# pyani-plus/pyani-plus

Hardware: AMD Instinct MI355X
Metric: pairwise genome comparisons/sec (N x N ANI matrix) (higher is better)
Workload: dtype u64

## Files before the change

include/pyani_hip.h:

```cpp
#ifndef PYANI_HIP_H
#define PYANI_HIP_H

#include <stddef.h>
#include <stdint.h>

#ifdef __cplusplus
extern "C" {
#endif

#define PA_ABI_VERSION 5

#define PA_API __attribute__((visibility("default")))

typedef enum pa_status {
  PA_OK = 0,
  PA_E_INVALID = -1,
  PA_E_HIP = -2,
  PA_E_NOMEM = -3,
  PA_E_CAPACITY = -4,
  PA_E_NODEVICE = -5,
  PA_E_IO = -6
} pa_status;

typedef struct pa_ctx pa_ctx;

#define PA_ALIGN_BASES 64u
#define PA_MAX_K 64u

PA_API int pa_abi_version(void);
PA_API const char *pa_last_error(void);
PA_API int pa_device_count(void);
PA_API int pa_ctx_create(int device, pa_ctx **out);
PA_API void pa_ctx_destroy(pa_ctx *ctx);
PA_API int pa_ctx_set_stream(pa_ctx *ctx, void *hip_stream);
PA_API int pa_ctx_own_stream(pa_ctx *ctx);
PA_API int pa_ctx_sync(pa_ctx *ctx);
PA_API int pa_ctx_device_info(pa_ctx *ctx, char *name256, int *compute_units, uint64_t *global_mem);

PA_API int pa_dev_alloc(pa_ctx *ctx, uint64_t bytes, void **d_out);
PA_API int pa_dev_free(pa_ctx *ctx, void *d_ptr);
PA_API int pa_memcpy_h2d(pa_ctx *ctx, void *d_dst, const void *h_src, uint64_t bytes);
PA_API int pa_memcpy_d2h(pa_ctx *ctx, void *h_dst, const void *d_src, uint64_t bytes);
PA_API int pa_memset_d(pa_ctx *ctx, void *d_dst, int value, uint64_t bytes);

PA_API uint64_t pa_pack_bound(uint64_t n_text_bytes);
PA_API int pa_pack_fasta(const uint8_t *h_text, uint64_t n_text, uint32_t *h_packed, uint32_t *h_mask,
                  uint64_t cap_bases, uint64_t *n_bases, uint64_t *n_residues, uint64_t *n_records,
                  uint64_t *n_invalid);
PA_API int pa_pack_seq(const uint8_t *h_seq, uint64_t n_seq, uint32_t *h_packed, uint32_t *h_mask,
                uint64_t cap_bases, uint64_t *n_bases, uint64_t *n_invalid);

PA_API int pa_gunzip(const uint8_t *h_gz, uint64_t n_gz, uint8_t *h_out, uint64_t cap, uint64_t *n_out, int decoder);

typedef struct pa_fasta_batch pa_fasta_batch;
PA_API int pa_fasta_batch_load(const char *const *paths, uint32_t n, int threads, pa_fasta_batch **out);
PA_API int pa_fasta_batch_info(const pa_fasta_batch *batch, uint32_t i, char md5hex33[33], uint64_t *n_residues,
                        uint64_t *n_records, uint64_t *n_invalid, uint64_t *n_bases, uint64_t *n_text,
                        const char **description, const char **message, int *was_gzip);
PA_API int pa_fasta_batch_records(const pa_fasta_batch *batch, uint32_t i, const uint64_t **rec_start,
                           const uint64_t **rec_len, uint64_t *n_records);
PA_API uint64_t pa_fasta_batch_arena_bases(const pa_fasta_batch *batch);
PA_API int pa_fasta_batch_copy_arena(const pa_fasta_batch *batch, uint32_t *h_packed, uint32_t *h_mask,
                              uint64_t *h_genome_start);
PA_API void pa_fasta_batch_free(pa_fasta_batch *batch);

PA_API uint64_t pa_max_hash(uint64_t scaled);

PA_API int pa_arena_dirty(pa_ctx *ctx, const uint32_t *d_mask, uint64_t arena_bases, uint64_t *d_dirty);

PA_API int pa_sketch(pa_ctx *ctx, const uint32_t *d_packed, const uint32_t *d_mask, const uint64_t *d_dirty,
              uint64_t arena_bases, const uint64_t *h_genome_start, uint32_t n_genomes, uint32_t k, uint64_t max_hash,
              uint64_t *d_hashes, uint64_t cap_hashes, uint64_t *d_off, uint64_t *h_total);

PA_API int64_t pa_mask_runs(const uint32_t *h_mask, uint64_t arena_bases, uint64_t *h_run_start, uint64_t *h_run_len,
                            uint64_t cap);
PA_API int pa_mask_from_runs(pa_ctx *ctx, const uint64_t *h_run_start, const uint64_t *h_run_len, uint32_t n_runs,
                             uint32_t *d_mask, uint64_t arena_bases);
PA_API int pa_sketch_streamed(pa_ctx *ctx, const uint32_t *h_packed, const uint64_t *h_run_start,
                              const uint64_t *h_run_len, uint32_t n_runs, uint64_t arena_bases,
                              const uint64_t *h_genome_start, uint32_t n_genomes, uint32_t k, uint64_t max_hash,
                              uint32_t *d_packed, uint32_t *d_mask, uint64_t *d_dirty, uint64_t *d_hashes,
                              uint64_t cap_hashes, uint64_t *d_off, uint64_t *h_total);

#define PA_PAIRS_AUTO 0
#define PA_PAIRS_BITROW 1
#define PA_PAIRS_MERGE 2
#define PA_PAIRS_BITROW_HASH 3
PA_API int pa_pair_counts(pa_ctx *ctx, const uint64_t *d_hashes, const uint64_t *d_off, uint32_t n,
                   uint32_t q0, uint32_t q1, uint32_t s0, uint32_t s1, uint32_t *d_counts, int algo);
PA_API int pa_pair_counts_ex(pa_ctx *ctx, const uint64_t *d_hashes, const uint64_t *d_off, const uint64_t *h_off,
                      uint32_t n, uint32_t q0, uint32_t q1, uint32_t s0, uint32_t s1, uint32_t *d_counts, int algo);
PA_API int pa_pair_dict_prepare(pa_ctx *ctx, const uint64_t *d_subject_hashes, uint64_t n_postings);

PA_API int pa_ani(pa_ctx *ctx, const uint32_t *d_counts, const uint64_t *d_off, uint32_t q0, uint32_t q1,
           uint32_t s0, uint32_t s1, uint32_t k, double *d_identity, double *d_cov_query);
PA_API int pa_ani_host(const uint32_t *h_counts, const uint64_t *h_q_sizes, const uint64_t *h_s_sizes,
                uint32_t nq, uint32_t ns, uint32_t k, double *h_identity, double *h_cov_query,
                uint8_t *h_is_null, int symmetric, uint32_t n_threads);

PA_API int pa_sketch_bottom(pa_ctx *ctx, const uint32_t *d_packed, const uint32_t *d_mask, const uint64_t *d_dirty, uint64_t arena_bases,
                     const uint64_t *h_genome_start, uint32_t n_genomes, uint32_t k, uint32_t m, uint64_t *d_hashes,
                     uint64_t cap_hashes, uint64_t *d_off, uint64_t *h_total);
PA_API int pa_pair_mash(pa_ctx *ctx, const uint64_t *d_hashes, const uint64_t *d_off, uint32_t n, uint32_t q0, uint32_t q1,
                 uint32_t s0, uint32_t s1, uint32_t m, uint32_t *d_common, uint32_t *d_denom);
PA_API int pa_ani_mash(pa_ctx *ctx, const uint32_t *d_common, const uint32_t *d_denom, uint64_t n_pairs, uint32_t k,
                double *d_ani);

PA_API int pa_fragani(pa_ctx *ctx, const uint32_t *d_packed, const uint32_t *d_mask, uint64_t arena_bases,
               const uint64_t *h_contig_start, const uint32_t *h_contig_len, const uint32_t *h_contig_genome,
               uint32_t n_contigs, uint32_t n_genomes, uint32_t k, uint32_t frag_len, uint32_t ref0, uint32_t ref1,
               uint32_t *h_total_frags, uint32_t *h_matched, double *h_ident_sum);
#define PA_FRAGANI_REUSE_INDEX 1u
#define PA_FRAGANI_COLUMNS_ONLY 2u
PA_API int pa_fragani_ex(pa_ctx *ctx, const uint32_t *d_packed, const uint32_t *d_mask, uint64_t arena_bases,
                  const uint64_t *h_contig_start, const uint32_t *h_contig_len, const uint32_t *h_contig_genome,
                  uint32_t n_contigs, uint32_t n_genomes, uint32_t k, uint32_t frag_len, uint32_t qry0, uint32_t qry1,
                  uint32_t ref0, uint32_t ref1, uint32_t flags, uint32_t *h_total_frags, uint32_t *h_matched,
                  double *h_ident_sum);
PA_API int pa_fragani_workspace(pa_ctx *ctx, uint64_t *held_bytes, uint64_t *peak_bytes, uint64_t *cap_bytes);
PA_API int pa_fragani_set_workspace_cap(pa_ctx *ctx, uint64_t cap_bytes);
PA_API int64_t pa_text_ambiguous(const uint8_t *h_text, uint64_t n_text, int fasta, uint64_t *h_pos, uint8_t *h_byte,
                                 uint64_t cap);
PA_API int64_t pa_fasta_batch_ambiguous(const pa_fasta_batch *batch, uint64_t *h_pos, uint8_t *h_byte, uint64_t cap);
PA_API int pa_fragani_set_ambiguous(pa_ctx *ctx, const uint32_t *d_packed, const uint64_t *h_pos, const uint8_t *h_byte,
                                    uint64_t n);
PA_API int pa_fragani_sketch(pa_ctx *ctx, const uint32_t *d_packed, const uint32_t *d_mask, uint64_t arena_bases,
                      const uint64_t *h_contig_start, const uint32_t *h_contig_len, const uint32_t *h_contig_genome,
                      uint32_t n_contigs, uint32_t n_genomes, uint32_t k, uint32_t window, uint32_t *h_hash,
                      uint32_t *h_wpos, uint32_t *h_contig, uint64_t cap, uint64_t *n_out);
PA_API int pa_fragani_window(uint32_t k, uint32_t frag_len);
PA_API int pa_fragani_tables(uint32_t k, uint32_t s_max, uint32_t *h_min_hits, uint32_t *h_min_shared);
PA_API double pa_fragani_identity(uint32_t shared, uint32_t s, uint32_t k);
PA_API int64_t pa_fasta_records(const uint8_t *h_text, uint64_t n_text, uint64_t *h_rec_start, uint64_t *h_rec_len,
                         uint64_t cap);

PA_API int pa_write_sigs(uint32_t n_files, const char *const *paths, const char *const *heads, const char *const *mids,
                         const char *const *tails, uint32_t ksize, const uint64_t *h_mins, const uint64_t *h_off,
                         uint32_t n_threads);

#define PA_SIG_UNHANDLED 1
typedef struct pa_sig_batch pa_sig_batch;
PA_API int pa_read_sigs(const char *const *paths, uint32_t n, uint32_t ksize, uint64_t max_hash, uint32_t n_threads,
                        pa_sig_batch **out);
PA_API int pa_sig_batch_info(const pa_sig_batch *batch, uint32_t i, uint64_t *n_mins, const char **message);
PA_API int pa_sig_batch_copy(const pa_sig_batch *batch, uint64_t *h_mins, uint64_t *h_off);
PA_API void pa_sig_batch_free(pa_sig_batch *batch);

PA_API int pa_write_comparisons_json(const char *path, const char *prefix, const char *suffix,
                              const char *const *q_hashes, uint32_t nq, const char *const *s_hashes, uint32_t ns,
                              const double *h_identity, const double *h_cov_query, const uint8_t *h_is_null);

PA_API int pa_append_comparisons_json(const char *path, const char *suffix, int file_has_rows,
                               const char *const *q_hashes, uint32_t nq, const char *const *s_hashes, uint32_t ns,
                               const double *h_identity, const double *h_cov_query, const uint8_t *h_is_null);

PA_API int pa_append_comparisons_json_ex(const char *path, const char *suffix, int file_has_rows,
                                  const char *const *q_hashes, uint32_t nq, const char *const *s_hashes, uint32_t ns,
                                  const double *h_identity, const double *h_cov_query, const uint8_t *h_is_null,
                                  const int64_t *h_aln_length, const int64_t *h_sim_errors);

PA_API int pa_round_sig6(double *h_values, uint64_t n);

PA_API uint32_t pa_host_cpu_budget(void);

PA_API int pa_sqlite_insert_comparisons(const char *database, int64_t configuration_id, const char *uname_system,
                                        const char *uname_release, const char *uname_machine,
                                        const char *const *query_hashes, uint32_t n_queries,
                                        const char *const *subject_hashes, uint32_t n_subjects,
                                        const double *h_identity, const double *h_cov_query, const uint8_t *h_is_null,
                                        uint64_t *rows_inserted);

PA_API int pa_sqlite_insert_comparisons_ex(const char *database, int64_t configuration_id, const char *uname_system,
                                           const char *uname_release, const char *uname_machine,
                                           const char *const *query_hashes, uint32_t n_queries,
                                           const char *const *subject_hashes, uint32_t n_subjects,
                                           const double *h_identity, const double *h_cov_query, const uint8_t *h_is_null,
                                           const int64_t *h_aln_length, const int64_t *h_sim_errors,
                                           uint64_t *rows_inserted);

typedef struct pa_msa pa_msa;
PA_API int pa_msa_load(const char *path, int threads, pa_msa **out);
PA_API int pa_msa_info(const pa_msa *msa, uint32_t *n_records, uint64_t *max_len, char md5hex33[33], uint64_t *h_hist256);
PA_API int pa_msa_record(const pa_msa *msa, uint32_t i, const char **title, uint64_t *title_len, uint64_t *length);
PA_API int pa_msa_copy_rows(const pa_msa *msa, uint32_t r0, uint32_t r1, uint64_t row_stride, uint8_t *h_rows);
PA_API void pa_msa_free(pa_msa *msa);
PA_API uint64_t pa_msa_plane_words(uint32_t n_rows, uint64_t n_cols, uint32_t bits);
PA_API int pa_msa_pack(pa_ctx *ctx, const uint8_t *d_rows, uint64_t row_stride, uint32_t row0, uint32_t n_chunk_rows, uint32_t n_rows,
                       uint64_t n_cols, const uint8_t *h_code256, uint32_t bits, uint32_t *d_planes, uint32_t *d_nongap);
PA_API int pa_msa_pair_counts(pa_ctx *ctx, const uint32_t *d_planes, uint32_t n_rows, uint64_t n_cols, uint32_t bits, uint32_t q0,
                              uint32_t q1, uint32_t s0, uint32_t s1, int symmetric, uint32_t *d_match, uint32_t *d_both);
PA_API int pa_msa_metrics(const uint32_t *h_match, const uint32_t *h_both, const uint64_t *h_nq, const uint64_t *h_ns, uint64_t n_pairs,
                          double *h_identity, int64_t *h_aln_length, int64_t *h_sim_errors, double *h_cov_query,
                          double *h_cov_subject, uint32_t n_threads);
PA_API int pa_append_msa_json(const char *path, const char *suffix, int file_has_rows, const char *const *hashes, uint32_t n_hashes,
                              const uint32_t *q_idx, const uint32_t *s_idx, uint64_t n_rows, const double *identity,
                              const int64_t *aln_length, const int64_t *sim_errors, const double *cov_query, const double *cov_subject);

#define PA_AGG_MIN 0
#define PA_AGG_MAX 1
#define PA_AGG_MEAN 2
typedef struct pa_cliques pa_cliques;
PA_API int pa_classify_edges(pa_ctx *ctx, const double *d_score, const double *d_cov, uint32_t n, int agg_score, int agg_cov,
                             double cov_min, uint64_t cap_edges, uint32_t *d_i, uint32_t *d_j, double *d_edge_score,
                             double *d_edge_cov, uint64_t *n_edges);
PA_API int pa_classify_edges_host(const double *h_score, const double *h_cov, uint32_t n, int agg_score, int agg_cov, double cov_min,
                                  uint64_t cap_edges, uint32_t *h_i, uint32_t *h_j, double *h_edge_score, double *h_edge_cov,
                                  uint64_t *n_edges);
PA_API int pa_classify_tani_host(const double *h_hadamard, uint64_t n_cells, double *h_score);
PA_API int pa_classify_cliques(uint32_t n, uint64_t n_edges, const uint32_t *h_i, const uint32_t *h_j, const double *h_edge_score,
                               const double *h_edge_cov, pa_cliques **out);
PA_API int pa_cliques_info(const pa_cliques *cl, uint64_t *n_rows, uint64_t *n_members);
PA_API int pa_cliques_copy(const pa_cliques *cl, uint32_t *n_nodes, double *max_cov, double *min_score, double *max_score,
                           uint8_t *present, uint64_t *member_off, uint32_t *members);
PA_API void pa_cliques_free(pa_cliques *cl);

#define PA_PROF_KMER_HASH 0
#define PA_PROF_SKETCH_SORT 1
#define PA_PROF_PAIR_DICT 2
#define PA_PROF_PAIR_COUNT 3
#define PA_PROF_ANI 4
#define PA_PROF_FRAG_INDEX 5
#define PA_PROF_FRAG_SEED 6
#define PA_PROF_FRAG_MAP 7
#define PA_PROF_MSA_PACK 8
#define PA_PROF_MSA_PAIRS 9
#define PA_PROF_CLS_EDGES 10
#define PA_PROF_CLS_SORT 11
#define PA_PROF_NPHASES 12
PA_API int pa_prof_enable(pa_ctx *ctx, int on);
PA_API int pa_prof_reset(pa_ctx *ctx);
PA_API int pa_prof_get(pa_ctx *ctx, int phase, double *total_ms, uint64_t *launches);

#ifdef __cplusplus
}
#endif
#endif
```

pyani_plus_amd/_capi.py:

```python

from __future__ import annotations

import ctypes as C
import os
import subprocess
from pathlib import Path

_PKG = Path(__file__).resolve().parent
LIB_PATH = _PKG / "_lib" / "libpyani_hip.so"
TOOLS_LIB_PATH = _PKG / "_lib" / "libpyani_hip_tools.so"

ABI_VERSION = 5
PA_OK = 0
PA_E_NOMEM = -3
PA_E_CAPACITY = -4
PA_E_IO = -6
PA_SIG_UNHANDLED = 1
PA_FRAGANI_REUSE_INDEX = 1
PA_FRAGANI_COLUMNS_ONLY = 2
PA_PAIRS_AUTO, PA_PAIRS_BITROW, PA_PAIRS_MERGE, PA_PAIRS_BITROW_HASH = 0, 1, 2, 3
PA_ALIGN_BASES = 64
PROF_PHASES = {"kmer_hash": 0, "sketch_sort": 1, "pair_dict": 2, "pair_count": 3, "ani": 4, "frag_index": 5, "frag_seed": 6, "frag_map": 7,
               "msa_pack": 8, "msa_pairs": 9, "cls_edges": 10, "cls_sort": 11}
PA_AGG = {"min": 0, "max": 1, "mean": 2}

_u8p = C.POINTER(C.c_uint8)
_u32p = C.POINTER(C.c_uint32)
_u64p = C.POINTER(C.c_uint64)
_f64p = C.POINTER(C.c_double)
_vp = C.c_void_p

SIGNATURES: dict[str, tuple] = {
    "pa_abi_version": (C.c_int, []),
    "pa_last_error": (C.c_char_p, []),
    "pa_device_count": (C.c_int, []),
    "pa_ctx_create": (C.c_int, [C.c_int, C.POINTER(_vp)]),
    "pa_ctx_destroy": (None, [_vp]),
    "pa_ctx_set_stream": (C.c_int, [_vp, _vp]),
    "pa_ctx_own_stream": (C.c_int, [_vp]),
    "pa_ctx_sync": (C.c_int, [_vp]),
    "pa_ctx_device_info": (C.c_int, [_vp, C.c_char_p, C.POINTER(C.c_int), _u64p]),
    "pa_dev_alloc": (C.c_int, [_vp, C.c_uint64, C.POINTER(_vp)]),
    "pa_dev_free": (C.c_int, [_vp, _vp]),
    "pa_memcpy_h2d": (C.c_int, [_vp, _vp, _vp, C.c_uint64]),
    "pa_memcpy_d2h": (C.c_int, [_vp, _vp, _vp, C.c_uint64]),
    "pa_memset_d": (C.c_int, [_vp, _vp, C.c_int, C.c_uint64]),
    "pa_pack_bound": (C.c_uint64, [C.c_uint64]),
    "pa_pack_fasta": (C.c_int, [_vp, C.c_uint64, _vp, _vp, C.c_uint64, _u64p, _u64p, _u64p, _u64p]),
    "pa_pack_seq": (C.c_int, [_vp, C.c_uint64, _vp, _vp, C.c_uint64, _u64p, _u64p]),
    "pa_max_hash": (C.c_uint64, [C.c_uint64]),
    "pa_fasta_batch_load": (C.c_int, [C.POINTER(C.c_char_p), C.c_uint32, C.c_int, C.POINTER(_vp)]),
    "pa_fasta_batch_info": (
        C.c_int,
        [_vp, C.c_uint32, C.c_char_p, _u64p, _u64p, _u64p, _u64p, _u64p, C.POINTER(C.c_char_p), C.POINTER(C.c_char_p), C.POINTER(C.c_int)],
    ),
    "pa_fasta_batch_records": (C.c_int, [_vp, C.c_uint32, C.POINTER(_u64p), C.POINTER(_u64p), _u64p]),
    "pa_fasta_batch_arena_bases": (C.c_uint64, [_vp]),
    "pa_fasta_batch_copy_arena": (C.c_int, [_vp, _vp, _vp, _vp]),
    "pa_fasta_batch_free": (None, [_vp]),
    "pa_arena_dirty": (C.c_int, [_vp, _vp, C.c_uint64, _vp]),
    "pa_sketch": (
        C.c_int,
        [_vp, _vp, _vp, _vp, C.c_uint64, _u64p, C.c_uint32, C.c_uint32, C.c_uint64, _vp, C.c_uint64, _vp, _u64p],
    ),
    "pa_read_sigs": (C.c_int, [C.POINTER(C.c_char_p), C.c_uint32, C.c_uint32, C.c_uint64, C.c_uint32, C.POINTER(_vp)]),
    "pa_sig_batch_info": (C.c_int, [_vp, C.c_uint32, _u64p, C.POINTER(C.c_char_p)]),
    "pa_sig_batch_copy": (C.c_int, [_vp, _vp, _vp]),
    "pa_sig_batch_free": (None, [_vp]),
    "pa_write_sigs": (C.c_int, [C.c_uint32, _vp, _vp, _vp, _vp, C.c_uint32, _vp, _vp, C.c_uint32]),
    "pa_mask_runs": (C.c_int64, [_vp, C.c_uint64, _vp, _vp, C.c_uint64]),
    "pa_mask_from_runs": (C.c_int, [_vp, _vp, _vp, C.c_uint32, _vp, C.c_uint64]),
    "pa_sketch_streamed": (
        C.c_int,
        [_vp, _vp, _vp, _vp, C.c_uint32, C.c_uint64, _u64p, C.c_uint32, C.c_uint32, C.c_uint64, _vp, _vp, _vp, _vp, C.c_uint64, _vp, _u64p],
    ),
    "pa_pair_counts": (
        C.c_int,
        [_vp, _vp, _vp, C.c_uint32, C.c_uint32, C.c_uint32, C.c_uint32, C.c_uint32, _vp, C.c_int],
    ),
    "pa_pair_counts_ex": (
        C.c_int,
        [_vp, _vp, _vp, _vp, C.c_uint32, C.c_uint32, C.c_uint32, C.c_uint32, C.c_uint32, _vp, C.c_int],
    ),
    "pa_pair_dict_prepare": (C.c_int, [_vp, _vp, C.c_uint64]),
    "pa_ani": (C.c_int, [_vp, _vp, _vp, C.c_uint32, C.c_uint32, C.c_uint32, C.c_uint32, C.c_uint32, _vp, _vp]),
    "pa_ani_host": (C.c_int, [_vp, _vp, _vp, C.c_uint32, C.c_uint32, C.c_uint32, _vp, _vp, _vp, C.c_int, C.c_uint32]),
    "pa_sketch_bottom": (
        C.c_int,
        [_vp, _vp, _vp, _vp, C.c_uint64, _u64p, C.c_uint32, C.c_uint32, C.c_uint32, _vp, C.c_uint64, _vp, _u64p],
    ),
    "pa_pair_mash": (C.c_int, [_vp, _vp, _vp, C.c_uint32, C.c_uint32, C.c_uint32, C.c_uint32, C.c_uint32, C.c_uint32, _vp, _vp]),
    "pa_ani_mash": (C.c_int, [_vp, _vp, _vp, C.c_uint64, C.c_uint32, _vp]),
    "pa_fragani": (C.c_int, [_vp, _vp, _vp, C.c_uint64, _vp, _vp, _vp, C.c_uint32, C.c_uint32, C.c_uint32, C.c_uint32, C.c_uint32, C.c_uint32, _vp, _vp, _vp]),
    "pa_fragani_ex": (
        C.c_int,
        [_vp, _vp, _vp, C.c_uint64, _vp, _vp, _vp, C.c_uint32, C.c_uint32, C.c_uint32, C.c_uint32, C.c_uint32, C.c_uint32, C.c_uint32,
         C.c_uint32, C.c_uint32, _vp, _vp, _vp],
    ),
    "pa_fragani_sketch": (
        C.c_int,
        [_vp, _vp, _vp, C.c_uint64, _vp, _vp, _vp, C.c_uint32, C.c_uint32, C.c_uint32, C.c_uint32, _vp, _vp, _vp, C.c_uint64, _u64p],
    ),
    "pa_text_ambiguous": (C.c_int64, [_vp, C.c_uint64, C.c_int, _vp, _vp, C.c_uint64]),
    "pa_fasta_batch_ambiguous": (C.c_int64, [_vp, _vp, _vp, C.c_uint64]),
    "pa_fragani_set_ambiguous": (C.c_int, [_vp, _vp, _vp, _vp, C.c_uint64]),
    "pa_fragani_window": (C.c_int, [C.c_uint32, C.c_uint32]),
    "pa_fragani_workspace": (C.c_int, [_vp, _u64p, _u64p, _u64p]),
    "pa_fragani_set_workspace_cap": (C.c_int, [_vp, C.c_uint64]),
    "pa_fragani_tables": (C.c_int, [C.c_uint32, C.c_uint32, _vp, _vp]),
    "pa_fragani_identity": (C.c_double, [C.c_uint32, C.c_uint32, C.c_uint32]),
    "pa_fasta_records": (C.c_int64, [_vp, C.c_uint64, _vp, _vp, C.c_uint64]),
    "pa_write_comparisons_json": (
        C.c_int,
        [C.c_char_p, C.c_char_p, C.c_char_p, C.POINTER(C.c_char_p), C.c_uint32, C.POINTER(C.c_char_p), C.c_uint32, _vp, _vp, _vp],
    ),
    "pa_append_comparisons_json": (
        C.c_int,
        [C.c_char_p, C.c_char_p, C.c_int, C.POINTER(C.c_char_p), C.c_uint32, C.POINTER(C.c_char_p), C.c_uint32, _vp, _vp, _vp],
    ),
    "pa_append_comparisons_json_ex": (
        C.c_int,
        [C.c_char_p, C.c_char_p, C.c_int, C.POINTER(C.c_char_p), C.c_uint32, C.POINTER(C.c_char_p), C.c_uint32, _vp, _vp, _vp, _vp, _vp],
    ),
    "pa_round_sig6": (C.c_int, [_vp, C.c_uint64]),
    "pa_host_cpu_budget": (C.c_uint32, []),
    "pa_gunzip": (C.c_int, [_vp, C.c_uint64, _vp, C.c_uint64, _u64p, C.c_int]),
    "pa_sqlite_insert_comparisons": (
        C.c_int,
        [C.c_char_p, C.c_int64, C.c_char_p, C.c_char_p, C.c_char_p, C.POINTER(C.c_char_p), C.c_uint32, C.POINTER(C.c_char_p), C.c_uint32, _vp, _vp, _vp, _u64p],
    ),
    "pa_sqlite_insert_comparisons_ex": (
        C.c_int,
        [C.c_char_p, C.c_int64, C.c_char_p, C.c_char_p, C.c_char_p, C.POINTER(C.c_char_p), C.c_uint32, C.POINTER(C.c_char_p), C.c_uint32, _vp, _vp, _vp,
         _vp, _vp, _u64p],
    ),
    "pa_msa_load": (C.c_int, [C.c_char_p, C.c_int, C.POINTER(_vp)]),
    "pa_msa_info": (C.c_int, [_vp, _u32p, _u64p, C.c_char_p, _u64p]),
    "pa_msa_record": (C.c_int, [_vp, C.c_uint32, C.POINTER(C.c_char_p), _u64p, _u64p]),
    "pa_msa_copy_rows": (C.c_int, [_vp, C.c_uint32, C.c_uint32, C.c_uint64, _vp]),
    "pa_msa_free": (None, [_vp]),
    "pa_msa_plane_words": (C.c_uint64, [C.c_uint32, C.c_uint64, C.c_uint32]),
    "pa_msa_pack": (C.c_int, [_vp, _vp, C.c_uint64, C.c_uint32, C.c_uint32, C.c_uint32, C.c_uint64, _vp, C.c_uint32, _vp, _vp]),
    "pa_msa_pair_counts": (
        C.c_int,
        [_vp, _vp, C.c_uint32, C.c_uint64, C.c_uint32, C.c_uint32, C.c_uint32, C.c_uint32, C.c_uint32, C.c_int, _vp, _vp],
    ),
    "pa_msa_metrics": (C.c_int, [_vp, _vp, _vp, _vp, C.c_uint64, _vp, _vp, _vp, _vp, _vp, C.c_uint32]),
    "pa_append_msa_json": (
        C.c_int,
        [C.c_char_p, C.c_char_p, C.c_int, C.POINTER(C.c_char_p), C.c_uint32, _vp, _vp, C.c_uint64, _vp, _vp, _vp, _vp, _vp],
    ),
    "pa_classify_edges": (C.c_int, [_vp, _vp, _vp, C.c_uint32, C.c_int, C.c_int, C.c_double, C.c_uint64, _vp, _vp, _vp, _vp, _u64p]),
    "pa_classify_edges_host": (C.c_int, [_vp, _vp, C.c_uint32, C.c_int, C.c_int, C.c_double, C.c_uint64, _vp, _vp, _vp, _vp, _u64p]),
    "pa_classify_tani_host": (C.c_int, [_vp, C.c_uint64, _vp]),
    "pa_classify_cliques": (C.c_int, [C.c_uint32, C.c_uint64, _vp, _vp, _vp, _vp, C.POINTER(_vp)]),
    "pa_cliques_info": (C.c_int, [_vp, _u64p, _u64p]),
    "pa_cliques_copy": (C.c_int, [_vp, _vp, _vp, _vp, _vp, _vp, _vp, _vp]),
    "pa_cliques_free": (None, [_vp]),
    "pa_prof_enable": (C.c_int, [_vp, C.c_int]),
    "pa_prof_reset": (C.c_int, [_vp]),
    "pa_prof_get": (C.c_int, [_vp, C.c_int, _f64p, _u64p]),
}


class HipBackendError(RuntimeError):
    """The HIP extension is missing, failed to load, or a call into it failed."""


_libs: dict[bool, C.CDLL] = {}


def build_library(force: bool = False) -> Path:
    srcdir = _PKG / "csrc"
    cmd = ["make", "-C", str(srcdir), "-j", str(min(8, os.cpu_count() or 1))]
    if force:
        cmd.append("-B")
    proc = subprocess.run(cmd, capture_output=True, text=True)
    if proc.returncode != 0 or not LIB_PATH.is_file() or not TOOLS_LIB_PATH.is_file():
        raise HipBackendError(f"building libpyani_hip.so failed:\n{proc.stdout}\n{proc.stderr}")
    return LIB_PATH


def load_library(tools: bool = False) -> C.CDLL:
    if tools in _libs:
        return _libs[tools]
    path = TOOLS_LIB_PATH if tools else LIB_PATH
    if not path.is_file():
        raise HipBackendError(
            f"{path} not found: build it with `python -c 'import __graft_entry__ as g; g.build()'` "
            "(or `make -C pyani_plus_amd/csrc`).  There is no CPU fallback for the compute path."
        )
    try:
        import torch
    except ImportError:
        pass
    try:
        lib = C.CDLL(str(path))
    except OSError as err:
        raise HipBackendError(f"cannot load {path}: {err}") from err
    for name, (restype, argtypes) in SIGNATURES.items():
        try:
            fn = getattr(lib, name)
        except AttributeError as err:
            raise HipBackendError(f"{path} does not export {name}") from err
        fn.restype = restype
        fn.argtypes = argtypes
    if lib.pa_abi_version() != ABI_VERSION:
        raise HipBackendError(f"ABI version mismatch: library reports {lib.pa_abi_version()}, binding expects {ABI_VERSION}")
    _libs[tools] = lib
    return lib


def last_error(lib: C.CDLL | None = None) -> str:
    return ((lib or load_library()).pa_last_error() or b"").decode(errors="replace")


def check(status: int, what: str, lib: C.CDLL | None = None) -> None:
    if status != PA_OK:
        err = HipBackendError(f"{what} failed with status {status}: {last_error(lib)}")
        err.status = status
        raise err
```

pyani_plus_amd/csrc/capi.hip:

```cpp
#include <algorithm>
#include <cstdarg>
#include <cstring>

#include "pa_internal.h"

static thread_local char g_err[1024] = "";

void pa_set_error(const char *fmt, ...) {
  va_list ap;
  va_start(ap, fmt);
  vsnprintf(g_err, sizeof(g_err), fmt, ap);
  va_end(ap);
}

static hipEvent_t take_event(pa_ctx *c) {
  if (!c->event_pool.empty()) {
    hipEvent_t e = c->event_pool.back();
    c->event_pool.pop_back();
    return e;
  }
  hipEvent_t e = nullptr;
  if (hipEventCreate(&e) != hipSuccess) return nullptr;
  return e;
}

ProfScope::ProfScope(pa_ctx *ctx, int ph) : c(ctx), phase(ph) {
  if (!c->prof_on) return;
  e0 = take_event(c);
  e1 = take_event(c);
  if (e0) (void)hipEventRecord(e0, c->stream);
}

ProfScope::~ProfScope() {
  if (!c->prof_on || !e0 || !e1) return;
  (void)hipEventRecord(e1, c->stream);
  c->prof[phase].pending.emplace_back(e0, e1);
}

extern "C" {

int pa_abi_version(void) { return PA_ABI_VERSION; }
const char *pa_last_error(void) { return g_err; }

int pa_device_count(void) {
  int n = 0;
  if (hipGetDeviceCount(&n) != hipSuccess) return 0;
  return n;
}

int pa_ctx_create(int device, pa_ctx **out) {
  PA_REQUIRE(out != nullptr, "pa_ctx_create: out is null");
  *out = nullptr;
  int n = 0;
  hipError_t e = hipGetDeviceCount(&n);
  if (e != hipSuccess || n <= 0) {
    pa_set_error("no HIP device available (%s); libpyani_hip has no CPU fallback",
                 e != hipSuccess ? hipGetErrorString(e) : "device count is 0");
    return PA_E_NODEVICE;
  }
  PA_REQUIRE(device >= 0 && device < n, "pa_ctx_create: device %d out of range [0,%d)", device, n);
  PA_HIP(hipSetDevice(device));
  pa_ctx *c = new (std::nothrow) pa_ctx();
  if (!c) { pa_set_error("out of host memory"); return PA_E_NOMEM; }
  c->device = device;
  if (hipGetDeviceProperties(&c->prop, device) != hipSuccess) { delete c; pa_set_error("hipGetDeviceProperties failed"); return PA_E_HIP; }
  if (strncmp(c->prop.gcnArchName, "gfx950", 6) != 0) {
    pa_set_error("device %d is %s; this library is built for gfx950 (MI355X) only", device, c->prop.gcnArchName);
    delete c;
    return PA_E_NODEVICE;
  }
  if (hipStreamCreateWithFlags(&c->stream, hipStreamNonBlocking) != hipSuccess) { delete c; pa_set_error("hipStreamCreate failed"); return PA_E_HIP; }
  c->own_stream = true;
  if (hipHostMalloc(reinterpret_cast<void **>(&c->h_pinned), 64, hipHostMallocDefault) != hipSuccess) {
    (void)hipStreamDestroy(c->stream); delete c; pa_set_error("hipHostMalloc failed"); return PA_E_NOMEM;
  }
  if (c->counters.reserve(64) != PA_OK) { (void)hipHostFree(c->h_pinned); (void)hipStreamDestroy(c->stream); delete c; return PA_E_NOMEM; }
  *out = c;
  return PA_OK;
}

void pa_ctx_destroy(pa_ctx *c) {
  if (!c) return;
  (void)hipSetDevice(c->device);
  (void)hipStreamSynchronize(c->stream);
  DevBuf *bufs[] = {&c->cand_keys[0], &c->cand_keys[1], &c->cand_vals[0], &c->cand_vals[1], &c->genome_blk,
                    &c->counters, &c->hist, &c->flags, &c->scan_tmp, &c->region_off, &c->region_cursor, &c->dirty, &c->dict_keys[0], &c->dict_keys[1],
                    &c->dict_vals[0], &c->dict_vals[1], &c->ids, &c->post_genome, &c->bitrows, &c->dict_scalars, &c->cls_i, &c->cls_j, &c->cls_score,
                    &c->cls_cov};
  for (DevBuf *b : bufs) b->release();
  pa_fragani_release(c);
  for (auto &ph : c->prof)
    for (auto &pr : ph.pending) { (void)hipEventDestroy(pr.first); (void)hipEventDestroy(pr.second); }
  for (hipEvent_t e : c->event_pool) (void)hipEventDestroy(e);
  if (c->h_pinned) (void)hipHostFree(c->h_pinned);
  if (c->copy_stream) { (void)hipStreamSynchronize(c->copy_stream); (void)hipStreamDestroy(c->copy_stream); c->copy_stream = nullptr; }
  if (c->own_stream && c->stream) (void)hipStreamDestroy(c->stream);
  delete c;
}

int pa_ctx_set_stream(pa_ctx *c, void *hip_stream) {
  PA_REQUIRE(c != nullptr, "null context");
  PA_HIP(hipStreamSynchronize(c->stream));
  if (c->own_stream && c->stream) (void)hipStreamDestroy(c->stream);
  c->stream = reinterpret_cast<hipStream_t>(hip_stream);
  c->own_stream = false;
  return PA_OK;
}

int pa_ctx_own_stream(pa_ctx *c) {
  PA_REQUIRE(c != nullptr, "null context");
  if (c->own_stream) return PA_OK;
  PA_HIP(hipStreamSynchronize(c->stream));
  PA_HIP(hipStreamCreateWithFlags(&c->stream, hipStreamNonBlocking));
  c->own_stream = true;
  return PA_OK;
}

int pa_ctx_sync(pa_ctx *c) {
  PA_REQUIRE(c != nullptr, "null context");
  PA_HIP(hipStreamSynchronize(c->stream));
  return PA_OK;
}

int pa_ctx_device_info(pa_ctx *c, char *name256, int *compute_units, uint64_t *global_mem) {
  PA_REQUIRE(c != nullptr, "null context");
  if (name256) { snprintf(name256, 256, "%s (%s)", c->prop.name, c->prop.gcnArchName); }
  if (compute_units) *compute_units = c->prop.multiProcessorCount;
  if (global_mem) *global_mem = (uint64_t)c->prop.totalGlobalMem;
  return PA_OK;
}

int pa_dev_alloc(pa_ctx *c, uint64_t bytes, void **d_out) {
  PA_REQUIRE(c && d_out, "pa_dev_alloc: null argument");
  PA_HIP(hipSetDevice(c->device));
  hipError_t e = hipMalloc(d_out, bytes ? bytes : 16);
  if (e != hipSuccess) { pa_set_error("hipMalloc(%llu) failed: %s", (unsigned long long)bytes, hipGetErrorString(e)); return PA_E_NOMEM; }
  return PA_OK;
}
int pa_dev_free(pa_ctx *c, void *d_ptr) {
  PA_REQUIRE(c != nullptr, "null context");
  if (d_ptr) { PA_HIP(hipStreamSynchronize(c->stream)); PA_HIP(hipFree(d_ptr)); }
  return PA_OK;
}
int pa_memcpy_h2d(pa_ctx *c, void *d_dst, const void *h_src, uint64_t bytes) {
  PA_REQUIRE(c != nullptr, "null context");
  if (bytes == 0) return PA_OK;
  PA_HIP(hipMemcpyAsync(d_dst, h_src, bytes, hipMemcpyHostToDevice, c->stream));
  PA_HIP(hipStreamSynchronize(c->stream));
  return PA_OK;
}
int pa_memcpy_d2h(pa_ctx *c, void *h_dst, const void *d_src, uint64_t bytes) {
  PA_REQUIRE(c != nullptr, "null context");
  if (bytes == 0) return PA_OK;
  PA_HIP(hipMemcpyAsync(h_dst, d_src, bytes, hipMemcpyDeviceToHost, c->stream));
  PA_HIP(hipStreamSynchronize(c->stream));
  return PA_OK;
}
int pa_memset_d(pa_ctx *c, void *d_dst, int value, uint64_t bytes) {
  PA_REQUIRE(c != nullptr, "null context");
  if (bytes == 0) return PA_OK;
  PA_HIP(hipMemsetAsync(d_dst, value, bytes, c->stream));
  return PA_OK;
}

int pa_sketch(pa_ctx *c, const uint32_t *d_packed, const uint32_t *d_mask, const uint64_t *d_dirty_in, uint64_t arena_bases,
              const uint64_t *h_genome_start, uint32_t n_genomes, uint32_t k, uint64_t max_hash, uint64_t *d_hashes,
              uint64_t cap_hashes, uint64_t *d_off, uint64_t *h_total) {
  PA_REQUIRE(c && d_off && h_total && h_genome_start, "pa_sketch: null argument");
  PA_REQUIRE((arena_bases % PA_ALIGN_BASES) == 0, "pa_sketch: arena_bases %llu is not a multiple of %u",
             (unsigned long long)arena_bases, PA_ALIGN_BASES);
  PA_REQUIRE(arena_bases == 0 || (d_packed && d_mask), "pa_sketch: null arena");
  PA_REQUIRE(k >= 1 && k <= PA_MAX_K, "pa_sketch: k=%u outside [1,%u]", k, PA_MAX_K);
  PA_REQUIRE(h_genome_start[n_genomes] == arena_bases, "pa_sketch: genome_start[n] must equal arena_bases");
  PA_HIP(hipSetDevice(c->device));
  *h_total = 0;
  const uint64_t n_blocks = arena_bases / PA_ALIGN_BASES;
  std::vector<uint32_t> blk(n_genomes + 1);
  for (uint32_t g = 0; g <= n_genomes; ++g) {
    const uint64_t s = h_genome_start[g];
    PA_REQUIRE((s % PA_ALIGN_BASES) == 0 && (g == 0 || s >= h_genome_start[g - 1]) && s <= arena_bases,
               "pa_sketch: genome_start[%u]=%llu must be an ascending multiple of %u inside the arena", g,
               (unsigned long long)s, PA_ALIGN_BASES);
    blk[g] = (uint32_t)(s / PA_ALIGN_BASES);
  }
  PA_REQUIRE(n_blocks < (1ULL << 32), "pa_sketch: arena too large");
  PA_TRY(c->genome_blk.reserve((uint64_t)(n_genomes + 1) * sizeof(uint32_t)));
  PA_HIP(hipMemcpyAsync(c->genome_blk.p, blk.data(), (uint64_t)(n_genomes + 1) * sizeof(uint32_t),
                        hipMemcpyHostToDevice, c->stream));
  const double frac = (max_hash == UINT64_MAX) ? 1.0 : ((double)max_hash + 1.0) / 18446744073709551616.0;
  static const bool force_global = [] {
    const char *v = PA_TOOL_ENV("PA_SKETCH_SORT");
    return v && v[0] == 'g';
  }();
  std::vector<uint64_t> region_off(n_genomes + 1, 0);
  uint64_t longest_region = 0;
  for (uint32_t g = 0; g < n_genomes; ++g) {
    const uint64_t room = (uint64_t)((double)(h_genome_start[g + 1] - h_genome_start[g]) * frac * 1.25) + 128;
    longest_region = std::max(longest_region, room);
    region_off[g + 1] = region_off[g] + room;
  }
  const bool use_regions = !force_global && n_genomes > 0 && longest_region <= kLdsSortMax;
  if (use_regions) {
    PA_TRY(c->region_off.reserve((uint64_t)(n_genomes + 1) * sizeof(uint64_t)));
    PA_TRY(c->region_cursor.reserve((uint64_t)n_genomes * sizeof(uint32_t)));
    PA_HIP(hipMemcpyAsync(c->region_off.p, region_off.data(), (uint64_t)(n_genomes + 1) * sizeof(uint64_t),
                          hipMemcpyHostToDevice, c->stream));
  }
  const uint64_t *d_dirty = nullptr;
  PA_TRY(pa_dirty_or_build(c, d_mask, n_blocks, d_dirty_in, &d_dirty));
  PA_HIP(hipStreamSynchronize(c->stream));

  if (use_regions) {
    uint32_t *d_overflow = c->counters.as<uint32_t>() + 12;
    PA_TRY(c->cand_keys[0].reserve(region_off[n_genomes] * sizeof(uint64_t)));
    PA_HIP(hipMemsetAsync(c->region_cursor.p, 0, (uint64_t)n_genomes * sizeof(uint32_t), c->stream));
    PA_HIP(hipMemsetAsync(d_overflow, 0, sizeof(uint32_t), c->stream));
    {
      ProfScope prof(c, PA_PROF_KMER_HASH);
      PA_TRY(pa_launch_kmer_hash(c, d_packed, d_mask, d_dirty, n_blocks, c->genome_blk.as<uint32_t>(), n_genomes, k, max_hash,
                                 c->cand_keys[0].as<uint64_t>(), nullptr, 0, nullptr, c->region_off.as<uint64_t>(),
                                 c->region_cursor.as<uint32_t>(), d_overflow));
    }
    bool overflow = false;
    {
      ProfScope prof(c, PA_PROF_SKETCH_SORT);
      const int st = pa_sketch_from_regions(c, c->cand_keys[0].as<uint64_t>(), c->region_off.as<uint64_t>(),
                                            c->region_cursor.as<uint32_t>(), d_overflow, n_genomes,
                                            (uint32_t)longest_region, max_hash, d_hashes, cap_hashes, d_off, h_total, &overflow);
      if (st != PA_OK) return st;
    }
    if (!overflow) return PA_OK;
    *h_total = 0;
  }
  uint64_t cap = (uint64_t)((double)arena_bases * frac * 1.25) + 65536;
  if (cap > arena_bases) cap = arena_bases;
  uint64_t *d_count = c->counters.as<uint64_t>();
  uint64_t n_cand = 0;
  for (int attempt = 0; attempt < 2; ++attempt) {
    for (int b = 0; b < 2; ++b) {
      PA_TRY(c->cand_keys[b].reserve(cap * sizeof(uint64_t)));
      PA_TRY(c->cand_vals[b].reserve(cap * sizeof(uint32_t)));
    }
    PA_HIP(hipMemsetAsync(d_count, 0, sizeof(uint64_t), c->stream));
    {
      ProfScope prof(c, PA_PROF_KMER_HASH);
      PA_TRY(pa_launch_kmer_hash(c, d_packed, d_mask, d_dirty, n_blocks, c->genome_blk.as<uint32_t>(), n_genomes, k, max_hash,
                                 c->cand_keys[0].as<uint64_t>(), c->cand_vals[0].as<uint32_t>(), cap, d_count));
    }
    PA_HIP(hipMemcpyAsync(c->h_pinned, d_count, sizeof(uint64_t), hipMemcpyDeviceToHost, c->stream));
    PA_HIP(hipStreamSynchronize(c->stream));
    n_cand = c->h_pinned[0];
    if (n_cand <= cap) break;
    PA_REQUIRE(attempt == 0, "pa_sketch: candidate count changed between runs (%llu > %llu)",
               (unsigned long long)n_cand, (unsigned long long)cap);
    cap = n_cand;
  }
  {
    ProfScope prof(c, PA_PROF_SKETCH_SORT);
    uint64_t *keys[2] = {c->cand_keys[0].as<uint64_t>(), c->cand_keys[1].as<uint64_t>()};
    uint32_t *vals[2] = {c->cand_vals[0].as<uint32_t>(), c->cand_vals[1].as<uint32_t>()};
    int which = 0;
    int hash_bits = max_hash ? 64 - __builtin_clzll(max_hash) : 0;
    hash_bits = (hash_bits + 7) & ~7;
    int genome_bits = n_genomes > 1 ? 32 - __builtin_clz(n_genomes - 1) : 0;
    genome_bits = (genome_bits + 7) & ~7;
    PA_TRY(pa_radix_sort_pairs(c, keys, vals, n_cand, 0, hash_bits, false, &which));
    PA_TRY(pa_radix_sort_pairs(c, keys, vals, n_cand, 0, genome_bits, true, &which));
    int st = pa_build_sketch_csr(c, keys[which], vals[which], n_cand, n_genomes, d_hashes, cap_hashes, d_off, h_total);
    if (st != PA_OK) return st;
  }
  return PA_OK;
}

int pa_pair_counts_ex(pa_ctx *c, const uint64_t *d_hashes, const uint64_t *d_off, const uint64_t *h_off, uint32_t n,
                      uint32_t q0, uint32_t q1, uint32_t s0, uint32_t s1, uint32_t *d_counts, int algo) {
  PA_REQUIRE(c && d_off, "pa_pair_counts: null argument");
  PA_REQUIRE(q0 <= q1 && q1 <= n && s0 <= s1 && s1 <= n, "pa_pair_counts: ranges [%u,%u) x [%u,%u) outside [0,%u)", q0,
             q1, s0, s1, n);
  PA_REQUIRE(algo == PA_PAIRS_AUTO || algo == PA_PAIRS_BITROW || algo == PA_PAIRS_MERGE || algo == PA_PAIRS_BITROW_HASH,
             "pa_pair_counts: unknown algo %d", algo);
  PA_HIP(hipSetDevice(c->device));
  if (q0 == q1 || s0 == s1) { c->dict_prepared = false; return PA_OK; }
  PA_REQUIRE(d_counts != nullptr, "pa_pair_counts: null counts buffer");
  uint64_t total = 0;
  if (h_off) {
    total = h_off[n];
  } else {
    PA_HIP(hipMemcpyAsync(c->h_pinned, d_off + n, sizeof(uint64_t), hipMemcpyDeviceToHost, c->stream));
    PA_HIP(hipStreamSynchronize(c->stream));
    total = c->h_pinned[0];
  }
  PA_REQUIRE(total == 0 || d_hashes, "pa_pair_counts: null hashes");
  if (algo != PA_PAIRS_AUTO && algo != PA_PAIRS_BITROW_HASH) c->dict_prepared = false;
  switch (algo) {
    case PA_PAIRS_AUTO:
    case PA_PAIRS_BITROW_HASH:
      return pa_pairs_bitrow_hash(c, d_hashes, d_off, h_off, n, total, q0, q1, s0, s1, d_counts);
    case PA_PAIRS_BITROW:
      return pa_pairs_bitrow(c, d_hashes, d_off, n, total, q0, q1, s0, s1, d_counts);
    case PA_PAIRS_MERGE:
      return pa_pairs_merge(c, d_hashes, d_off, n, q0, q1, s0, s1, d_counts);
    default:
      pa_set_error("pa_pair_counts: unknown algo %d", algo);
      return PA_E_INVALID;
  }
}

int pa_pair_counts(pa_ctx *c, const uint64_t *d_hashes, const uint64_t *d_off, uint32_t n, uint32_t q0, uint32_t q1,
                   uint32_t s0, uint32_t s1, uint32_t *d_counts, int algo) {
  return pa_pair_counts_ex(c, d_hashes, d_off, nullptr, n, q0, q1, s0, s1, d_counts, algo);
}

int pa_pair_dict_prepare(pa_ctx *c, const uint64_t *d_subject_hashes, uint64_t n_postings) {
  PA_REQUIRE(c && (n_postings == 0 || d_subject_hashes), "pa_pair_dict_prepare: null argument");
  PA_HIP(hipSetDevice(c->device));
  return pa_pair_dict_prepare_impl(c, d_subject_hashes, n_postings);
}

int pa_ani(pa_ctx *c, const uint32_t *d_counts, const uint64_t *d_off, uint32_t q0, uint32_t q1, uint32_t s0,
           uint32_t s1, uint32_t k, double *d_identity, double *d_cov_query) {
  PA_REQUIRE(c && d_counts && d_off && d_identity && d_cov_query, "pa_ani: null argument");
  PA_REQUIRE(k >= 1 && q0 <= q1 && s0 <= s1, "pa_ani: bad k or ranges");
  PA_HIP(hipSetDevice(c->device));
  return pa_launch_ani(c, d_counts, d_off, q0, q1, s0, s1, k, d_identity, d_cov_query);
}

int pa_prof_enable(pa_ctx *c, int on) {
  PA_REQUIRE(c != nullptr, "null context");
  c->prof_on = on != 0;
  return PA_OK;
}

static int prof_drain(pa_ctx *c) {
  PA_HIP(hipStreamSynchronize(c->stream));
  for (auto &ph : c->prof) {
    for (auto &pr : ph.pending) {
      float ms = 0.f;
      if (hipEventElapsedTime(&ms, pr.first, pr.second) == hipSuccess) {
        ph.total_ms += ms;
        ph.launches += 1;
      }
      c->event_pool.push_back(pr.first);
      c->event_pool.push_back(pr.second);
    }
    ph.pending.clear();
  }
  return PA_OK;
}

int pa_prof_reset(pa_ctx *c) {
  PA_REQUIRE(c != nullptr, "null context");
  PA_TRY(prof_drain(c));
  for (auto &ph : c->prof) { ph.total_ms = 0.0; ph.launches = 0; }
  return PA_OK;
}

int pa_prof_get(pa_ctx *c, int phase, double *total_ms, uint64_t *launches) {
  PA_REQUIRE(c != nullptr && phase >= 0 && phase < PA_PROF_NPHASES, "pa_prof_get: bad phase %d", phase);
  PA_TRY(prof_drain(c));
  if (total_ms) *total_ms = c->prof[phase].total_ms;
  if (launches) *launches = c->prof[phase].launches;
  return PA_OK;
}

}
```

pyani_plus_amd/csrc/kmer_hash.hip:

```cpp
#include <cstdlib>
#include <type_traits>

#include "pa_internal.h"
#include "murmur_dev.h"

namespace {

using namespace pa_dev;

constexpr int kThreads = 256;
constexpr uint32_t kStageCap = 1024;

constexpr int pow2_floor(int k) { int c = 1; while (2 * c <= k) c *= 2; return c; }

__device__ __forceinline__ uint32_t find_genome(const uint32_t *__restrict__ genome_blk, uint32_t n, uint32_t blk) {
  uint32_t lo = 0, hi = n;
  while (hi - lo > 1) {
    uint32_t mid = (lo + hi) >> 1;
    if (genome_blk[mid] <= blk) lo = mid; else hi = mid;
  }
  return lo;
}

__device__ __forceinline__ void region_append(uint64_t *__restrict__ regions, const uint64_t *__restrict__ region_off,
                                              uint32_t *__restrict__ cursor, uint32_t *__restrict__ overflow,
                                              uint32_t g, uint64_t h) {
  const uint64_t slot = atomicAdd(&cursor[g], 1u);
  if (slot < region_off[g + 1] - region_off[g]) regions[region_off[g] + slot] = h; else *overflow = 1u;
}

template <int K, bool LUT>
__global__ __launch_bounds__(kThreads) void kmer_hash_kernel(
    const uint4 *__restrict__ packed, const uint2 *__restrict__ mask, const uint64_t *__restrict__ dirty, uint32_t n_blocks64,
    const uint32_t *__restrict__ genome_blk, uint32_t n_genomes, uint64_t max_hash,
    uint64_t *__restrict__ cand_hash, uint32_t *__restrict__ cand_genome, uint64_t cap,
    unsigned long long *__restrict__ count, const uint64_t *__restrict__ region_off, uint32_t *__restrict__ cursor,
    uint32_t *__restrict__ overflow, uint32_t blk0) {
  static_assert(K >= 1 && K <= 32, "a k-mer is one 64-bit register pair");
  __shared__ uint64_t s_hash[kStageCap];
  __shared__ uint32_t s_blk[kStageCap];
  __shared__ uint32_t s_n;
  __shared__ unsigned long long s_base;
  constexpr int kWords = (K + 7) / 8;
  __shared__ uint64_t s_lo[LUT ? kWords : 1][256];
  __shared__ uint32_t s_hi[LUT ? kWords : 1][256];

  const uint32_t tid = threadIdx.x;
  const uint32_t max_hi = (uint32_t)(max_hash >> 32);
  const bool take_all = max_hi == 0xffffffffu;
  const uint32_t screen_hi = max_hi + 1u;
  if (tid == 0) s_n = 0;
  if constexpr (LUT) {
#pragma unroll
    for (int j = 0; j < kWords; ++j) {
      const uint64_t cj = (j & 1) ? kC2 : kC1;
      s_lo[j][tid] = (uint64_t)ascii_group(tid, K - 8 * j) * cj;
      s_hi[j][tid] = (uint32_t)((uint64_t)ascii_group(tid, K - 8 * j - 4) * cj);
    }
  }
  __syncthreads();

  const uint32_t t = blk0 + blockIdx.x * kThreads + tid;
  if (t < n_blocks64) {
    const uint4 cur = packed[t];
    uint2 pw = make_uint2(0u, 0u);
    if (t > 0) pw = reinterpret_cast<const uint2 *>(packed)[2 * (uint64_t)t - 1];
    uint32_t d1 = 0u, d2 = 0u;
    const uint32_t wave_blk = __builtin_amdgcn_readfirstlane(t & ~63u);
    const uint64_t dirty_word = dirty[wave_blk >> 6];
    if ((dirty_word >> (t & 63u)) & 1ull) {
      const uint2 m = mask[t];
      uint32_t d0 = t > 0 ? mask[t - 1].y : 0xffffffffu;
      d1 = m.x;
      d2 = m.y;
      int c = 1;
#pragma unroll
      for (; 2 * c <= K; c *= 2) {
        d2 |= alignbit(d2, d1, 32 - c);
        d1 |= alignbit(d1, d0, 32 - c);
        d0 |= d0 << c;
      }
      constexpr int cc = pow2_floor(K);
      constexpr int r = K - cc;
      if constexpr (r > 0) {
        d2 |= alignbit(d2, d1, 32 - r);
        d1 |= alignbit(d1, d0, 32 - r);
      }
    }
    const uint32_t bad[2] = {d1, d2};
    if ((d1 & d2) != 0xffffffffu) {
      constexpr uint64_t kMask = (K == 32) ? ~0ULL : ((1ULL << (2 * K)) - 1);
      constexpr uint32_t kMaskHi = (uint32_t)(kMask >> 32);
      uint32_t fw[8] = {pw.x, pw.y, cur.x, cur.y, cur.z, cur.w, 0u, 0u};
      uint32_t rw[6];
#pragma unroll
      for (int j = 0; j < 6; ++j) {
        const uint32_t x = __builtin_bitreverse32(fw[5 - j]);
        rw[j] = ~(((x >> 1) & 0x55555555u) | ((x & 0x55555555u) << 1));
      }
      auto columns = [&](auto base_tag, int i_begin, int i_end) {
        constexpr int kBase = decltype(base_tag)::value;
#pragma unroll 1
        for (int i = i_begin; i < i_end; ++i) {
          constexpr int kOff = 33 - K;
          const uint32_t fo = 2u * (uint32_t)((i + kOff) & 15), ro = 30u - 2u * (uint32_t)i;
          uint32_t A[5], B[5];
#pragma unroll
          for (int j = 0; j < 5; ++j) {
            A[j] = alignbit(fw[kBase + j + 1], fw[kBase + j], fo);
            B[j] = alignbit(rw[j + 1], rw[j], ro);
          }
#pragma unroll
          for (int wi = 0; wi < 4; ++wi) {
            const uint32_t f_lo = A[wi], f_hi = A[wi + 1], r_lo = B[3 - wi], r_hi = B[4 - wi];
          const uint64_t f_lsb = u64_of(f_lo, f_hi) & kMask, r_lsb = u64_of(r_lo, r_hi) & kMask;
          const uint64_t fwd = __builtin_amdgcn_uicmpl(f_lsb, r_lsb, 37 );
          uint32_t clo, chi;
          asm("s_nop 1\n\tv_cndmask_b32_e64 %0, %1, %2, %3" : "=v"(clo) : "v"((uint32_t)r_lsb), "v"((uint32_t)f_lsb), "s"(fwd));
          asm("v_cndmask_b32_e64 %0, %1, %2, %3" : "=v"(chi) : "v"((uint32_t)(r_lsb >> 32)), "v"((uint32_t)(f_lsb >> 32)), "s"(fwd), "v"(clo));
          uint64_t P[4] = {0, 0, 0, 0};
#pragma unroll
          for (int j = 0; j < kWords; ++j) {
            const uint32_t src = j < 2 ? clo : chi;
            const uint32_t glo = (src >> (16 * (j & 1))) & 0xffu, ghi = (src >> (16 * (j & 1) + 8)) & 0xffu;
            if constexpr (LUT) {
              const uint64_t lo = s_lo[j][glo];
              const uint32_t hi = (uint32_t)(lo >> 32) + s_hi[j][ghi];
              P[j] = u64_of((uint32_t)lo, hi);
            } else {
              const uint64_t word = u64_of(ascii_group(glo, K - 8 * j), ascii_group(ghi, K - 8 * j - 4));
              P[j] = word * ((j & 1) ? kC2 : kC1);
            }
          }
          (void)kMaskHi;
          uint64_t U, V;
          murmur3_pre_last_mul<K>(P, U, V);
          if (take_all || last_mul_high_sum_plus1(U, V) <= screen_hi) {
            const uint64_t X = U * kF2, Y = V * kF2;
            const uint64_t h = (X ^ (X >> 33)) + (Y ^ (Y >> 33));
            if (h > max_hash || ((bad[wi >> 1] >> (16 * (wi & 1) + i)) & 1u)) continue;
            const uint32_t slot = atomicAdd(&s_n, 1u);
            if (slot < kStageCap) {
              s_hash[slot] = h;
              s_blk[slot] = t;
            } else if (region_off) {
              region_append(cand_hash, region_off, cursor, overflow, find_genome(genome_blk, n_genomes, t), h);
            } else {
              const unsigned long long g = atomicAdd(count, 1ULL);
              if (g < cap) {
                cand_hash[g] = h;
                cand_genome[g] = find_genome(genome_blk, n_genomes, t);
              }
            }
          }
          }
        }
      };
      constexpr int kOff0 = 33 - K, kSplit = (kOff0 & 15) ? 16 - (kOff0 & 15) : 16;
      columns(std::integral_constant<int, (kOff0 >> 4)>{}, 0, kSplit);
      if constexpr (kSplit < 16) columns(std::integral_constant<int, (kOff0 >> 4) + 1>{}, kSplit, 16);
    }
  }
  __syncthreads();
  const uint32_t n = min(s_n, kStageCap);
  if (n == 0) return;
  if (region_off) {
    const uint32_t b0 = blk0 + blockIdx.x * kThreads;
    const uint32_t b1 = min(b0 + (uint32_t)kThreads, n_blocks64) - 1u;
    const uint32_t g0 = find_genome(genome_blk, n_genomes, b0);
    if (genome_blk[g0 + 1] > b1) {
      if (tid == 0) s_base = atomicAdd(&cursor[g0], n);
      __syncthreads();
      const uint64_t room = region_off[g0 + 1] - region_off[g0];
      uint64_t *__restrict__ dst = cand_hash + region_off[g0];
      for (uint32_t i = tid; i < n; i += kThreads) {
        const uint64_t slot = s_base + i;
        if (slot < room) dst[slot] = s_hash[i]; else *overflow = 1u;
      }
    } else {
      for (uint32_t i = tid; i < n; i += kThreads)
        region_append(cand_hash, region_off, cursor, overflow, find_genome(genome_blk, n_genomes, s_blk[i]), s_hash[i]);
    }
    return;
  }
  if (tid == 0) s_base = atomicAdd(count, (unsigned long long)n);
  __syncthreads();
  const unsigned long long base = s_base;
  for (uint32_t i = tid; i < n; i += kThreads) {
    const unsigned long long g = base + i;
    if (g < cap) {
      cand_hash[g] = s_hash[i];
      cand_genome[g] = find_genome(genome_blk, n_genomes, s_blk[i]);
    }
  }
}

template <int K, bool LUT>
int launch_variant(pa_ctx *c, const uint32_t *d_packed, const uint32_t *d_mask, const uint64_t *d_dirty, uint64_t n_blocks64,
           const uint32_t *d_genome_blk, uint32_t n_genomes, uint64_t max_hash, uint64_t *d_cand_hash,
           uint32_t *d_cand_genome, uint64_t cap, uint64_t *d_count, const uint64_t *d_region_off, uint32_t *d_cursor,
           uint32_t *d_overflow, uint64_t blk0, hipStream_t stream) {
  const uint32_t grid = ceil_div_u64(n_blocks64 - blk0, kThreads);
  hipLaunchKernelGGL((kmer_hash_kernel<K, LUT>), dim3(grid), dim3(kThreads), 0, stream ? stream : c->stream,
                     reinterpret_cast<const uint4 *>(d_packed), reinterpret_cast<const uint2 *>(d_mask), d_dirty,
                     (uint32_t)n_blocks64, d_genome_blk, n_genomes, max_hash, d_cand_hash, d_cand_genome, cap,
                     reinterpret_cast<unsigned long long *>(d_count), d_region_off, d_cursor, d_overflow, (uint32_t)blk0);
  PA_HIP(hipGetLastError());
  return PA_OK;
}

template <int K>
int launch(pa_ctx *c, const uint32_t *d_packed, const uint32_t *d_mask, const uint64_t *d_dirty, uint64_t n_blocks64,
           const uint32_t *d_genome_blk, uint32_t n_genomes, uint64_t max_hash, uint64_t *d_cand_hash,
           uint32_t *d_cand_genome, uint64_t cap, uint64_t *d_count, const uint64_t *d_region_off, uint32_t *d_cursor,
           uint32_t *d_overflow, uint64_t blk0, hipStream_t stream) {
  static const bool arithmetic = [] {
    const char *v = PA_TOOL_ENV("PA_KMER_VARIANT");
    return v && v[0] == '0';
  }();
  if constexpr (K == 31)
    if (arithmetic)
      return launch_variant<K, false>(c, d_packed, d_mask, d_dirty, n_blocks64, d_genome_blk, n_genomes, max_hash, d_cand_hash,
                                    d_cand_genome, cap, d_count, d_region_off, d_cursor, d_overflow, blk0, stream);
  return launch_variant<K, true>(c, d_packed, d_mask, d_dirty, n_blocks64, d_genome_blk, n_genomes, max_hash, d_cand_hash,
                                 d_cand_genome, cap, d_count, d_region_off, d_cursor, d_overflow, blk0, stream);
}

template <int K>
__global__ __launch_bounds__(kThreads) void kmer_hash_wide_kernel(
    const uint4 *__restrict__ packed, const uint2 *__restrict__ mask, const uint64_t *__restrict__ dirty, uint32_t n_blocks64,
    const uint32_t *__restrict__ genome_blk, uint32_t n_genomes, uint64_t max_hash,
    uint64_t *__restrict__ cand_hash, uint32_t *__restrict__ cand_genome, uint64_t cap,
    unsigned long long *__restrict__ count, const uint64_t *__restrict__ region_off, uint32_t *__restrict__ cursor,
    uint32_t *__restrict__ overflow, uint32_t blk0) {
  static_assert(K >= 33 && K <= 64, "k-mers of 65 to 128 bits");
  __shared__ uint64_t s_hash[kStageCap];
  __shared__ uint32_t s_blk[kStageCap];
  __shared__ uint32_t s_n;
  __shared__ unsigned long long s_base;
  constexpr int kWords = (K + 7) / 8;
  __shared__ uint64_t s_lo[kWords][256];
  __shared__ uint32_t s_hi[kWords][256];
  const uint32_t tid = threadIdx.x;
  const uint32_t max_hi = (uint32_t)(max_hash >> 32);
  const bool take_all = max_hi == 0xffffffffu;
  const uint32_t screen_hi = max_hi + 1u;
  if (tid == 0) s_n = 0;
#pragma unroll
  for (int j = 0; j < kWords; ++j) {
    const uint64_t cj = (j & 1) ? kC2 : kC1;
    s_lo[j][tid] = (uint64_t)ascii_group(tid, K - 8 * j) * cj;
    s_hi[j][tid] = (uint32_t)((uint64_t)ascii_group(tid, K - 8 * j - 4) * cj);
  }
  __syncthreads();

  const uint32_t t = blk0 + blockIdx.x * kThreads + tid;
  if (t < n_blocks64) {
    const uint4 cur = packed[t];
    const uint4 prev = t > 0 ? packed[t - 1] : make_uint4(0u, 0u, 0u, 0u);
    uint32_t d2 = 0u, d3 = 0u;
    const uint32_t wave_blk = __builtin_amdgcn_readfirstlane(t & ~63u);
    const uint64_t dirty_word = dirty[wave_blk >> 6];
    const uint64_t before = wave_blk ? dirty[(wave_blk >> 6) - 1] >> 63 : 1ull;
    const uint64_t dirty_or_prev = dirty_word | (dirty_word << 1) | before;
    if ((dirty_or_prev >> (t & 63u)) & 1ull) {
      const uint2 m = mask[t];
      uint32_t d0 = 0xffffffffu, d1 = 0xffffffffu;
      if (t > 0) { const uint2 mp = mask[t - 1]; d0 = mp.x; d1 = mp.y; }
      d2 = m.x;
      d3 = m.y;
#pragma unroll
      for (int c = 1; c <= 16; c *= 2) {
        d3 |= alignbit(d3, d2, 32 - c);
        d2 |= alignbit(d2, d1, 32 - c);
        d1 |= alignbit(d1, d0, 32 - c);
        d0 |= d0 << c;
      }
      if constexpr (K == 64) {
        d3 |= d2; d2 |= d1; d1 |= d0;
      } else {
        constexpr int r = K - 32;
        d3 |= alignbit(d3, d2, 32 - r);
        d2 |= alignbit(d2, d1, 32 - r);
        d1 |= alignbit(d1, d0, 32 - r);
      }
    }
    const uint32_t bad[2] = {d2, d3};
    if ((d2 & d3) != 0xffffffffu) {
      constexpr uint32_t kMask2 = (2 * K - 64 >= 32) ? 0xffffffffu : ((1u << (2 * K - 64)) - 1u);
      constexpr uint32_t kMask3 = (2 * K - 96 >= 32) ? 0xffffffffu : (2 * K - 96 <= 0 ? 0u : ((1u << ((2 * K - 96) & 31)) - 1u));
      const uint32_t fw[10] = {prev.x, prev.y, prev.z, prev.w, cur.x, cur.y, cur.z, cur.w, 0u, 0u};
      uint32_t rw[10];
#pragma unroll
      for (int j = 0; j < 10; ++j) {
        const uint32_t x = __builtin_bitreverse32(fw[9 - j]);
        rw[j] = ~(((x >> 1) & 0x55555555u) | ((x & 0x55555555u) << 1));
      }
      auto columns = [&](auto base_tag, int i_begin, int i_end) {
        constexpr int kBase = decltype(base_tag)::value;
#pragma unroll 1
        for (int i = i_begin; i < i_end; ++i) {
          constexpr int kOff = 65 - K;
          const uint32_t fo = 2u * (uint32_t)((i + kOff) & 15), ro = 30u - 2u * (uint32_t)i;
          uint32_t A[7], B[7];
#pragma unroll
          for (int j = 0; j < 7; ++j) {
            A[j] = alignbit(fw[kBase + j + 1], fw[kBase + j], fo);
            B[j] = alignbit(rw[j + 3], rw[j + 2], ro);
          }
#pragma unroll
          for (int wi = 0; wi < 4; ++wi) {
            const uint32_t f0 = A[wi], f1 = A[wi + 1], f2 = A[wi + 2] & kMask2, f3 = A[wi + 3] & kMask3;
            const uint32_t r0 = B[3 - wi], r1 = B[4 - wi], r2 = B[5 - wi] & kMask2, r3 = B[6 - wi] & kMask3;
            const uint64_t lt_hi = __builtin_amdgcn_uicmpl(u64_of(f2, f3), u64_of(r2, r3), 36 );
            const uint64_t eq_hi = __builtin_amdgcn_uicmpl(u64_of(f2, f3), u64_of(r2, r3), 32 );
            const uint64_t le_lo = __builtin_amdgcn_uicmpl(u64_of(f0, f1), u64_of(r0, r1), 37 );
            const uint64_t fwd = lt_hi | (eq_hi & le_lo);
            uint32_t c0, c1, c2, c3;
            asm("s_nop 1\n\tv_cndmask_b32_e64 %0, %1, %2, %3" : "=v"(c0) : "v"(r0), "v"(f0), "s"(fwd));
            asm("v_cndmask_b32_e64 %0, %1, %2, %3" : "=v"(c1) : "v"(r1), "v"(f1), "s"(fwd), "v"(c0));
            asm("v_cndmask_b32_e64 %0, %1, %2, %3" : "=v"(c2) : "v"(r2), "v"(f2), "s"(fwd), "v"(c1));
            asm("v_cndmask_b32_e64 %0, %1, %2, %3" : "=v"(c3) : "v"(r3), "v"(f3), "s"(fwd), "v"(c2));
            const uint32_t cw[4] = {c0, c1, c2, c3};
            uint64_t P[8] = {0, 0, 0, 0, 0, 0, 0, 0};
#pragma unroll
            for (int j = 0; j < kWords; ++j) {
              const uint32_t src = cw[j >> 1];
              const uint32_t glo = (src >> (16 * (j & 1))) & 0xffu, ghi = (src >> (16 * (j & 1) + 8)) & 0xffu;
              const uint64_t lo = s_lo[j][glo];
              P[j] = u64_of((uint32_t)lo, (uint32_t)(lo >> 32) + s_hi[j][ghi]);
            }
            uint64_t U, V;
            murmur3_pre_last_mul<K>(P, U, V);
            if (take_all || last_mul_high_sum_plus1(U, V) <= screen_hi) {
              const uint64_t X = U * kF2, Y = V * kF2;
              const uint64_t h = (X ^ (X >> 33)) + (Y ^ (Y >> 33));
              if (h > max_hash || ((bad[wi >> 1] >> (16 * (wi & 1) + i)) & 1u)) continue;
              const uint32_t slot = atomicAdd(&s_n, 1u);
              if (slot < kStageCap) {
                s_hash[slot] = h;
                s_blk[slot] = t;
              } else if (region_off) {
                region_append(cand_hash, region_off, cursor, overflow, find_genome(genome_blk, n_genomes, t), h);
              } else {
                const unsigned long long g = atomicAdd(count, 1ULL);
                if (g < cap) {
                  cand_hash[g] = h;
                  cand_genome[g] = find_genome(genome_blk, n_genomes, t);
                }
              }
            }
          }
        }
      };
      constexpr int kOff0 = 65 - K, kSplit = (kOff0 & 15) ? 16 - (kOff0 & 15) : 16;
      columns(std::integral_constant<int, (kOff0 >> 4)>{}, 0, kSplit);
      if constexpr (kSplit < 16) columns(std::integral_constant<int, (kOff0 >> 4) + 1>{}, kSplit, 16);
    }
  }
  __syncthreads();
  const uint32_t n = min(s_n, kStageCap);
  if (n == 0) return;
  if (region_off) {
    const uint32_t b0 = blk0 + blockIdx.x * kThreads;
    const uint32_t b1 = min(b0 + (uint32_t)kThreads, n_blocks64) - 1u;
    const uint32_t g0 = find_genome(genome_blk, n_genomes, b0);
    if (genome_blk[g0 + 1] > b1) {
      if (tid == 0) s_base = atomicAdd(&cursor[g0], n);
      __syncthreads();
      const uint64_t room = region_off[g0 + 1] - region_off[g0];
      uint64_t *__restrict__ dst = cand_hash + region_off[g0];
      for (uint32_t i = tid; i < n; i += kThreads) {
        const uint64_t slot = s_base + i;
        if (slot < room) dst[slot] = s_hash[i]; else *overflow = 1u;
      }
    } else {
      for (uint32_t i = tid; i < n; i += kThreads)
        region_append(cand_hash, region_off, cursor, overflow, find_genome(genome_blk, n_genomes, s_blk[i]), s_hash[i]);
    }
    return;
  }
  if (tid == 0) s_base = atomicAdd(count, (unsigned long long)n);
  __syncthreads();
  const unsigned long long base = s_base;
  for (uint32_t i = tid; i < n; i += kThreads) {
    const unsigned long long g = base + i;
    if (g < cap) {
      cand_hash[g] = s_hash[i];
      cand_genome[g] = find_genome(genome_blk, n_genomes, s_blk[i]);
    }
  }
}

__device__ __forceinline__ uint32_t rev_groups32(uint32_t x) {
  x = __builtin_bitreverse32(x);
  return ((x >> 1) & 0x55555555u) | ((x & 0x55555555u) << 1);
}

__device__ __forceinline__ void murmur3_pre_last_mul_rt(const uint64_t (&P)[8], uint32_t k, uint64_t &U, uint64_t &V) {
  uint64_t h1 = 42, h2 = 42;
  const uint32_t nblocks = k >> 4, tail = k & 15u;
#pragma unroll
  for (uint32_t i = 0; i < 4; ++i) {
    if (i >= nblocks) break;
    h1 ^= rotl64(P[2 * i], 31) * kC2;
    h1 = rotl64(h1, 27) + h2;
    h1 = times5_plus(h1, 0x52dce729ULL);
    h2 ^= rotl64(P[2 * i + 1], 33) * kC1;
    h2 = rotl64(h2, 31) + h1;
    h2 = times5_plus(h2, 0x38495ab5ULL);
  }
  uint64_t t1 = 0, t2 = 0;
#pragma unroll
  for (uint32_t i = 0; i < 4; ++i)
    if (i == nblocks) { t1 = P[2 * i]; t2 = P[2 * i + 1]; }
  if (tail > 8) h2 ^= rotl64(t2, 33) * kC1;
  if (tail > 0) h1 ^= rotl64(t1, 31) * kC2;
  h1 ^= (uint64_t)k;
  h2 ^= (uint64_t)k;
  h1 += h2;
  h2 += h1;
  h1 ^= h1 >> 33; h1 *= kF1; h1 ^= h1 >> 33;
  h2 ^= h2 >> 33; h2 *= kF1; h2 ^= h2 >> 33;
  U = h1;
  V = h2;
}

constexpr int kLongIter = 32;
__global__ __launch_bounds__(kThreads) void kmer_hash_long_kernel(
    const uint32_t *__restrict__ packed, const uint32_t *__restrict__ mask, uint64_t pos0, uint64_t pos1, uint32_t k,
    const uint32_t *__restrict__ genome_blk, uint32_t n_genomes, uint64_t max_hash, uint64_t *__restrict__ cand_hash,
    uint32_t *__restrict__ cand_genome, uint64_t cap, unsigned long long *__restrict__ count,
    const uint64_t *__restrict__ region_off, uint32_t *__restrict__ cursor, uint32_t *__restrict__ overflow) {
  __shared__ uint64_t s_lo[8][256];
  __shared__ uint32_t s_hi[8][256];
  const uint32_t tid = threadIdx.x;
  const uint32_t n_words = (k + 7u) >> 3;
  for (uint32_t j = 0; j < n_words; ++j) {
    const uint64_t cj = (j & 1u) ? kC2 : kC1;
    s_lo[j][tid] = (uint64_t)ascii_group(tid, (int)k - 8 * (int)j) * cj;
    s_hi[j][tid] = (uint32_t)((uint64_t)ascii_group(tid, (int)k - 8 * (int)j - 4) * cj);
  }
  __syncthreads();
  const uint64_t wg_first = pos0 + ((uint64_t)blockIdx.y * gridDim.x + blockIdx.x) * (uint64_t)(kThreads * kLongIter);
#pragma unroll 1
  for (int it = 0; it < kLongIter; ++it) {
  const uint64_t e = wg_first + (uint64_t)it * kThreads + tid;
  if (e >= pos1 || e + 1 < k) continue;
  const uint64_t a = e + 1 - k;
  {
    const uint64_t m0 = a >> 5, m_last = e >> 5;
    const uint32_t sm = (uint32_t)(a & 31u);
    const uint32_t w0 = mask[m0], w1 = m0 + 1 <= m_last ? mask[m0 + 1] : 0u, w2 = m0 + 2 <= m_last ? mask[m0 + 2] : 0u;
    const uint32_t b0 = alignbit(w1, w0, sm), b1 = alignbit(w2, w1, sm);
    const uint32_t top = k == 64 ? 0xffffffffu : ((1u << (k - 32u)) - 1u);
    if (b0 | (b1 & top)) continue;
  }
  uint32_t F[4], R[4];
  {
    const uint64_t p0 = a >> 4, p_last = e >> 4;
    const uint32_t sp = 2u * (uint32_t)(a & 15u);
    uint32_t w[5];
#pragma unroll
    for (int i = 0; i < 5; ++i) w[i] = p0 + i <= p_last ? packed[p0 + i] : 0u;
#pragma unroll
    for (int i = 0; i < 4; ++i) F[i] = alignbit(w[i + 1], w[i], sp);
    const uint32_t used = 2u * k - 64u;
    if (used < 32u) { F[2] &= (1u << used) - 1u; F[3] = 0u; }
    else if (used < 64u) F[3] &= (1u << (used - 32u)) - 1u;
    const uint32_t C[6] = {~rev_groups32(F[3]), ~rev_groups32(F[2]), ~rev_groups32(F[1]), ~rev_groups32(F[0]), 0u, 0u};
    const uint32_t s = 128u - 2u * k, ws = s >> 5, bs = s & 31u;
#pragma unroll
    for (int i = 0; i < 4; ++i) R[i] = ws ? alignbit(C[i + 2], C[i + 1], bs) : alignbit(C[i + 1], C[i], bs);
    if (used < 32u) { R[2] &= (1u << used) - 1u; R[3] = 0u; }
    else if (used < 64u) R[3] &= (1u << (used - 32u)) - 1u;
  }
  const uint64_t f_hi = u64_of(F[2], F[3]), f_lo = u64_of(F[0], F[1]), r_hi = u64_of(R[2], R[3]), r_lo = u64_of(R[0], R[1]);
  const bool fwd = f_hi < r_hi || (f_hi == r_hi && f_lo <= r_lo);
  uint32_t c[4];
#pragma unroll
  for (int i = 0; i < 4; ++i) c[i] = fwd ? F[i] : R[i];
  uint64_t P[8] = {0, 0, 0, 0, 0, 0, 0, 0};
#pragma unroll
  for (uint32_t j = 0; j < 8; ++j) {
    if (j >= n_words) break;
    const uint32_t src = c[j >> 1], glo = (src >> (16u * (j & 1u))) & 0xffu, ghi = (src >> (16u * (j & 1u) + 8u)) & 0xffu;
    const uint64_t lo = s_lo[j][glo];
    P[j] = u64_of((uint32_t)lo, (uint32_t)(lo >> 32) + s_hi[j][ghi]);
  }
  uint64_t U, V;
  murmur3_pre_last_mul_rt(P, k, U, V);
  const uint32_t max_hi = (uint32_t)(max_hash >> 32);
  if (max_hi != 0xffffffffu && last_mul_high_sum_plus1(U, V) > max_hi + 1u) continue;
  const uint64_t X = U * kF2, Y = V * kF2;
  const uint64_t h = (X ^ (X >> 33)) + (Y ^ (Y >> 33));
  if (h > max_hash) continue;
  const uint32_t blk = (uint32_t)(e >> 6);
  const uint32_t g = find_genome(genome_blk, n_genomes, blk);
  if (region_off) {
    region_append(cand_hash, region_off, cursor, overflow, g, h);
  } else {
    const unsigned long long slot = atomicAdd(count, 1ULL);
    if (slot < cap) {
      cand_hash[slot] = h;
      cand_genome[slot] = g;
    }
  }
  }
}

}

int pa_launch_kmer_hash(pa_ctx *c, const uint32_t *d_packed, const uint32_t *d_mask, const uint64_t *d_dirty, uint64_t n_blocks64,
                        const uint32_t *d_genome_blk, uint32_t n_genomes, uint32_t k, uint64_t max_hash,
                        uint64_t *d_cand_hash, uint32_t *d_cand_genome, uint64_t cap, uint64_t *d_count,
                        const uint64_t *d_region_off, uint32_t *d_cursor, uint32_t *d_overflow, uint64_t blk0,
                        hipStream_t stream) {
  PA_REQUIRE(n_blocks64 < (1ULL << 32), "arena too large: %llu blocks of 64 bases", (unsigned long long)n_blocks64);
  if (n_blocks64 <= blk0) return PA_OK;
  const char *long_form = PA_TOOL_ENV("PA_KMER_LONG");
  const bool long_plain = long_form && long_form[0] == 'p';
  if (k > 32 && k <= 64 && !long_plain) {
    PA_REQUIRE((blk0 & 63u) == 0, "k-mer hash launch must start at a multiple of 64 blocks, not %llu", (unsigned long long)blk0);
    const uint32_t grid = ceil_div_u64(n_blocks64 - blk0, kThreads);
#define PA_WIDE_CASE(KK)                                                                                                   \
  case KK:                                                                                                                 \
    hipLaunchKernelGGL((kmer_hash_wide_kernel<KK>), dim3(grid), dim3(kThreads), 0, stream ? stream : c->stream,            \
                       reinterpret_cast<const uint4 *>(d_packed), reinterpret_cast<const uint2 *>(d_mask), d_dirty,        \
                       (uint32_t)n_blocks64, d_genome_blk, n_genomes, max_hash, d_cand_hash, d_cand_genome, cap,           \
                       reinterpret_cast<unsigned long long *>(d_count), d_region_off, d_cursor, d_overflow, (uint32_t)blk0); \
    break;
    switch (k) {
      PA_WIDE_CASE(33) PA_WIDE_CASE(34) PA_WIDE_CASE(35) PA_WIDE_CASE(36) PA_WIDE_CASE(37) PA_WIDE_CASE(38) PA_WIDE_CASE(39)
      PA_WIDE_CASE(40) PA_WIDE_CASE(41) PA_WIDE_CASE(42) PA_WIDE_CASE(43) PA_WIDE_CASE(44) PA_WIDE_CASE(45) PA_WIDE_CASE(46)
      PA_WIDE_CASE(47) PA_WIDE_CASE(48) PA_WIDE_CASE(49) PA_WIDE_CASE(50) PA_WIDE_CASE(51) PA_WIDE_CASE(52) PA_WIDE_CASE(53)
      PA_WIDE_CASE(54) PA_WIDE_CASE(55) PA_WIDE_CASE(56) PA_WIDE_CASE(57) PA_WIDE_CASE(58) PA_WIDE_CASE(59) PA_WIDE_CASE(60)
      PA_WIDE_CASE(61) PA_WIDE_CASE(62) PA_WIDE_CASE(63) PA_WIDE_CASE(64)
      default: break;
    }
#undef PA_WIDE_CASE
    PA_HIP(hipGetLastError());
    return PA_OK;
  }
  if (k > 32 && k <= 64) {
    const uint64_t pos0 = blk0 * 64, pos1 = n_blocks64 * 64;
    const uint64_t per_wg = (uint64_t)kThreads * kLongIter;
    const uint64_t n_wg = (pos1 - pos0 + per_wg - 1) / per_wg;
    const uint32_t gx = (uint32_t)std::min<uint64_t>(n_wg, 1u << 20), gy = (uint32_t)((n_wg + gx - 1) / gx);
    PA_REQUIRE(gy <= 65535u, "arena too large for one launch of the long k-mer kernel: %llu positions", (unsigned long long)(pos1 - pos0));
    hipLaunchKernelGGL(kmer_hash_long_kernel, dim3(gx, gy), dim3(kThreads), 0,
                       stream ? stream : c->stream, d_packed, d_mask, pos0, pos1, k, d_genome_blk, n_genomes, max_hash,
                       d_cand_hash, d_cand_genome, cap, reinterpret_cast<unsigned long long *>(d_count), d_region_off,
                       d_cursor, d_overflow);
    PA_HIP(hipGetLastError());
    return PA_OK;
  }
#define PA_K_CASE(KK) \
  case KK: return launch<KK>(c, d_packed, d_mask, d_dirty, n_blocks64, d_genome_blk, n_genomes, max_hash, d_cand_hash, d_cand_genome, cap, d_count, d_region_off, d_cursor, d_overflow, blk0, stream);
  PA_REQUIRE((blk0 & 63u) == 0, "k-mer hash launch must start at a multiple of 64 blocks, not %llu", (unsigned long long)blk0);
  switch (k) {
    PA_K_CASE(1) PA_K_CASE(2) PA_K_CASE(3) PA_K_CASE(4) PA_K_CASE(5) PA_K_CASE(6) PA_K_CASE(7) PA_K_CASE(8)
    PA_K_CASE(9) PA_K_CASE(10) PA_K_CASE(11) PA_K_CASE(12) PA_K_CASE(13) PA_K_CASE(14) PA_K_CASE(15) PA_K_CASE(16)
    PA_K_CASE(17) PA_K_CASE(18) PA_K_CASE(19) PA_K_CASE(20) PA_K_CASE(21) PA_K_CASE(22) PA_K_CASE(23) PA_K_CASE(24)
    PA_K_CASE(25) PA_K_CASE(26) PA_K_CASE(27) PA_K_CASE(28) PA_K_CASE(29) PA_K_CASE(30) PA_K_CASE(31) PA_K_CASE(32)
    default:
      pa_set_error("k=%u outside [1,64]", k);
      return PA_E_INVALID;
  }
#undef PA_K_CASE
}
```

pyani_plus_amd/csrc/murmur_dev.h:

```cpp
#pragma once

#include <hip/hip_runtime.h>

#include <cstdint>

namespace pa_dev {

__device__ __forceinline__ uint32_t alignbit(uint32_t hi, uint32_t lo, uint32_t sh) {
  return __builtin_amdgcn_alignbit(hi, lo, sh);
}

__device__ __forceinline__ uint32_t ascii4(uint32_t b8) {
  uint32_t u = (b8 | (b8 << 12)) & 0x000F000Fu;
  uint32_t v = (u | (u << 6)) & 0x03030303u;
  return __builtin_amdgcn_perm(0u, 0x54474341u, v);
}

__device__ __forceinline__ uint64_t u64_of(uint32_t lo, uint32_t hi) { return ((uint64_t)hi << 32) | lo; }

__device__ __forceinline__ uint64_t rotl64(uint64_t x, int r) {
  const uint32_t lo = (uint32_t)x, hi = (uint32_t)(x >> 32);
  if (r == 32) return u64_of(hi, lo);
  if (r < 32) return u64_of(alignbit(lo, hi, 32 - r), alignbit(hi, lo, 32 - r));
  return u64_of(alignbit(hi, lo, 64 - r), alignbit(lo, hi, 64 - r));
}

__device__ __forceinline__ uint64_t fmix64(uint64_t k) {
  k ^= k >> 33;
  k *= 0xff51afd7ed558ccdULL;
  k ^= k >> 33;
  k *= 0xc4ceb9fe1a85ec53ULL;
  k ^= k >> 33;
  return k;
}

constexpr uint64_t kC1 = 0x87c37b91114253d5ULL, kC2 = 0x4cf5ad432745937fULL;

__device__ __forceinline__ uint64_t times5_plus(uint64_t h, uint64_t c) {
  uint64_t t;
  asm("v_lshl_add_u64 %0, %1, 2, %1" : "=v"(t) : "v"(h));
  return t + c;
}

constexpr uint64_t kF1 = 0xff51afd7ed558ccdULL, kF2 = 0xc4ceb9fe1a85ec53ULL;

template <int K, int N>
__device__ __forceinline__ void murmur3_pre_last_mul(const uint64_t (&P)[N], uint64_t &U, uint64_t &V) {
  static_assert(N >= (K + 7) / 8, "one first product per 8-byte word of the k-mer");
  uint64_t h1 = 42, h2 = 42;
  constexpr int nblocks = K / 16;
  constexpr int tail = K % 16;
#pragma unroll
  for (int i = 0; i < nblocks; ++i) {
    const uint64_t k1 = rotl64(P[2 * i], 31) * kC2;
    h1 ^= k1;
    if (i == 0) {
      h1 = times5_plus(rotl64(h1, 27), 5ULL * 42ULL + 0x52dce729ULL);
    } else {
      h1 = rotl64(h1, 27) + h2;
      h1 = times5_plus(h1, 0x52dce729ULL);
    }
    const uint64_t k2 = rotl64(P[2 * i + 1], 33) * kC1;
    h2 ^= k2;
    h2 = rotl64(h2, 31) + h1;
    h2 = times5_plus(h2, 0x38495ab5ULL);
  }
  if constexpr (tail > 8) h2 ^= rotl64(P[2 * nblocks + 1], 33) * kC1;
  if constexpr (tail > 0) h1 ^= rotl64(P[2 * nblocks], 31) * kC2;
  h1 ^= (uint64_t)K; h2 ^= (uint64_t)K;
  h1 += h2; h2 += h1;
  h1 ^= h1 >> 33; h1 *= kF1; h1 ^= h1 >> 33;
  h2 ^= h2 >> 33; h2 *= kF1; h2 ^= h2 >> 33;
  U = h1;
  V = h2;
}

__device__ __forceinline__ uint32_t last_mul_high_sum_plus1(uint64_t U, uint64_t V) {
  constexpr uint32_t c0 = (uint32_t)kF2, c1 = (uint32_t)(kF2 >> 32);
  const uint32_t u0 = (uint32_t)U, u1 = (uint32_t)(U >> 32), v0 = (uint32_t)V, v1 = (uint32_t)(V >> 32);
  return (__umulhi(u0, c0) + __umulhi(v0, c0) + 1u) + ((u0 + v0) * c1 + (u1 + v1) * c0);
}

template <int K, int N>
__device__ __forceinline__ uint64_t murmur3_from_products(const uint64_t (&P)[N]) {
  uint64_t U, V;
  murmur3_pre_last_mul<K, N>(P, U, V);
  const uint64_t X = U * kF2, Y = V * kF2;
  return (X ^ (X >> 33)) + (Y ^ (Y >> 33));
}

__device__ __forceinline__ uint32_t ascii_group(uint32_t b8, int nv) {
  const uint32_t a = ascii4(b8);
  return nv >= 4 ? a : (nv <= 0 ? 0u : (a & ((1u << (8 * nv)) - 1u)));
}

}
```

pyani_plus_amd/csrc/pa_internal.h:

```cpp
#pragma once

#include <hip/hip_runtime.h>

#include <cstdarg>
#include <cstdint>
#include <cstdio>
#include <string>
#include <vector>

#include "../../include/pyani_hip.h"

void pa_set_error(const char *fmt, ...);

#define PA_HIP(call)                                                                          \
  do {                                                                                        \
    hipError_t _e = (call);                                                                   \
    if (_e != hipSuccess) {                                                                   \
      pa_set_error("%s failed: %s (%s:%d)", #call, hipGetErrorString(_e), __FILE__, __LINE__); \
      return PA_E_HIP;                                                                        \
    }                                                                                         \
  } while (0)

#define PA_TRY(call)          \
  do {                        \
    int _s = (call);          \
    if (_s != PA_OK) return _s; \
  } while (0)

#define PA_REQUIRE(cond, ...)   \
  do {                          \
    if (!(cond)) {              \
      pa_set_error(__VA_ARGS__); \
      return PA_E_INVALID;      \
    }                           \
  } while (0)

#ifdef PA_TOOLS
#include <cstdlib>
#define PA_TOOL_ENV(name) getenv(name)
#else
#define PA_TOOL_ENV(name) static_cast<const char *>(nullptr)
#endif

struct DevBudget {
  uint64_t held = 0, peak = 0, cap = 0;
  char what[192] = {0};
};
struct DevBuf {
  void *p = nullptr;
  uint64_t bytes = 0;
  DevBudget *budget = nullptr;
  int reserve(uint64_t want) {
    if (want <= bytes) return PA_OK;
    uint64_t sz = want + want / 4 + 256;
    if (budget && budget->cap && budget->held - bytes + sz > budget->cap) {
      pa_set_error("%s: the workspace would grow to %llu bytes (%llu held; this buffer from %llu to %llu), above the cap of %llu bytes",
                   budget->what[0] ? budget->what : "device workspace", (unsigned long long)(budget->held - bytes + sz),
                   (unsigned long long)budget->held, (unsigned long long)bytes, (unsigned long long)sz, (unsigned long long)budget->cap);
      return PA_E_NOMEM;
    }
    if (p) (void)hipFree(p);
    if (budget) budget->held -= bytes;
    p = nullptr;
    bytes = 0;
    hipError_t e = hipMalloc(&p, sz);
    if (e != hipSuccess) {
      if (budget)
        pa_set_error("%s: hipMalloc(%llu) failed with %llu bytes of workspace held: %s", budget->what[0] ? budget->what : "device workspace",
                     (unsigned long long)sz, (unsigned long long)budget->held, hipGetErrorString(e));
      else
        pa_set_error("hipMalloc(%llu) failed: %s", (unsigned long long)sz, hipGetErrorString(e));
      p = nullptr;
      return PA_E_NOMEM;
    }
    bytes = sz;
    if (budget) {
      budget->held += sz;
      if (budget->held > budget->peak) budget->peak = budget->held;
    }
    return PA_OK;
  }
  void release() {
    if (p) (void)hipFree(p);
    if (budget) budget->held -= bytes;
    p = nullptr;
    bytes = 0;
  }
  template <typename T>
  T *as() const { return reinterpret_cast<T *>(p); }
};

struct ProfPhase {
  double total_ms = 0.0;
  uint64_t launches = 0;
  std::vector<std::pair<hipEvent_t, hipEvent_t>> pending;
};

struct pa_ctx {
  int device = 0;
  hipStream_t stream = nullptr;
  bool own_stream = false;
  hipDeviceProp_t prop;
  DevBuf cand_keys[2], cand_vals[2];
  DevBuf genome_blk;
  DevBuf counters;
  DevBuf hist;
  DevBuf flags, scan_tmp;
  DevBuf region_off, region_cursor;
  DevBuf dirty;
  DevBuf dict_keys[2], dict_vals[2];
  DevBuf ids, post_genome, bitrows;
  bool dict_prepared = false;
  uint64_t dict_prepared_postings = 0;
  uint32_t dict_prepared_cap = 0;
  DevBuf dict_scalars;
  hipStream_t copy_stream = nullptr;
  DevBuf cls_i, cls_j, cls_score, cls_cov;
  void *frag_work = nullptr;
  uint64_t *h_pinned = nullptr;
  bool prof_on = false;
  ProfPhase prof[PA_PROF_NPHASES];
  std::vector<hipEvent_t> event_pool;
};

struct ProfScope {
  pa_ctx *c;
  int phase;
  hipEvent_t e0 = nullptr, e1 = nullptr;
  ProfScope(pa_ctx *ctx, int ph);
  ~ProfScope();
};

static inline uint32_t ceil_div_u64(uint64_t a, uint64_t b) { return (uint32_t)((a + b - 1) / b); }

int pa_radix_sort_pairs(pa_ctx *c, uint64_t *keys[2], uint32_t *vals[2], uint64_t n, int bit_lo,
                        int bit_hi, bool by_val, int *which);
int pa_exclusive_scan_u32(pa_ctx *c, const uint32_t *d_in, uint32_t *d_out, uint64_t n,
                          uint64_t *d_total_u64 );

void pa_fragani_release(pa_ctx *c);

int pa_launch_kmer_hash(pa_ctx *c, const uint32_t *d_packed, const uint32_t *d_mask, const uint64_t *d_dirty, uint64_t n_blocks64,
                        const uint32_t *d_genome_blk, uint32_t n_genomes, uint32_t k, uint64_t max_hash,
                        uint64_t *d_cand_hash, uint32_t *d_cand_genome, uint64_t cap, uint64_t *d_count,
                        const uint64_t *d_region_off = nullptr, uint32_t *d_cursor = nullptr,
                        uint32_t *d_overflow = nullptr, uint64_t blk0 = 0, hipStream_t stream = nullptr);

int pa_build_dirty(pa_ctx *c, const uint32_t *d_mask, uint64_t n_blocks64, uint64_t *d_dirty, hipStream_t stream = nullptr);
int pa_dirty_or_build(pa_ctx *c, const uint32_t *d_mask, uint64_t n_blocks64, const uint64_t *d_dirty, const uint64_t **out);

constexpr uint32_t kLdsSortMax = 16384;
int pa_sketch_from_regions(pa_ctx *c, uint64_t *d_regions, const uint64_t *d_region_off, const uint32_t *d_cursor,
                           const uint32_t *d_overflow, uint32_t n_genomes, uint32_t longest_region, uint64_t max_hash,
                           uint64_t *d_hashes, uint64_t cap_hashes, uint64_t *d_off, uint64_t *h_total, bool *h_overflow);

int pa_build_sketch_csr(pa_ctx *c, const uint64_t *d_sorted_hash, const uint32_t *d_sorted_genome,
                        uint64_t n_cand, uint32_t n_genomes, uint64_t *d_hashes, uint64_t cap_hashes,
                        uint64_t *d_off, uint64_t *h_total);

int pa_pairs_bitrow(pa_ctx *c, const uint64_t *d_hashes, const uint64_t *d_off, uint32_t n, uint64_t total,
                    uint32_t q0, uint32_t q1, uint32_t s0, uint32_t s1, uint32_t *d_counts);
int pa_dense_ids_sorted(pa_ctx *c, const uint64_t *d_hashes, const uint64_t *d_off, uint32_t n, uint64_t P,
                        uint64_t *n_distinct);
int pa_pairs_bitrow_hash(pa_ctx *c, const uint64_t *d_hashes, const uint64_t *d_off, const uint64_t *h_off ,
                         uint32_t n, uint64_t total, uint32_t q0, uint32_t q1, uint32_t s0, uint32_t s1,
                         uint32_t *d_counts);
int pa_pair_dict_prepare_impl(pa_ctx *c, const uint64_t *d_subject_hashes, uint64_t n_postings);
int pa_pairs_merge(pa_ctx *c, const uint64_t *d_hashes, const uint64_t *d_off, uint32_t n, uint32_t q0,
                   uint32_t q1, uint32_t s0, uint32_t s1, uint32_t *d_counts);

int pa_launch_ani(pa_ctx *c, const uint32_t *d_counts, const uint64_t *d_off, uint32_t q0, uint32_t q1,
                  uint32_t s0, uint32_t s1, uint32_t k, double *d_identity, double *d_cov_query);
```

pyani_plus_amd/csrc/sketch_build.hip:

```cpp
#include "pa_internal.h"

namespace {

constexpr int kThreads = 256;

__global__ __launch_bounds__(kThreads) void head_flags_kernel(const uint64_t *__restrict__ hash,
                                                              const uint32_t *__restrict__ genome, uint64_t n,
                                                              uint32_t *__restrict__ flags) {
  const uint64_t i = (uint64_t)blockIdx.x * kThreads + threadIdx.x;
  if (i >= n) return;
  flags[i] = (i == 0 || hash[i] != hash[i - 1] || genome[i] != genome[i - 1]) ? 1u : 0u;
}

__global__ __launch_bounds__(kThreads) void compact_csr_kernel(
    const uint64_t *__restrict__ hash, const uint32_t *__restrict__ genome, const uint32_t *__restrict__ flags,
    const uint32_t *__restrict__ pos, uint64_t n, uint32_t n_genomes, uint64_t cap, uint64_t *__restrict__ out_hash,
    uint64_t *__restrict__ off) {
  const uint64_t i = (uint64_t)blockIdx.x * kThreads + threadIdx.x;
  if (i >= n) return;
  const uint32_t g = genome[i];
  const uint32_t p = pos[i];
  if (flags[i]) {
    if (p < cap) out_hash[p] = hash[i];
    const int64_t gp = (i == 0) ? -1 : (int64_t)genome[i - 1];
    for (int64_t x = gp + 1; x <= (int64_t)g; ++x) off[x] = p;
  }
  if (i == n - 1) {
    const uint64_t total = (uint64_t)p + flags[i];
    for (uint32_t x = g + 1; x <= n_genomes; ++x) off[x] = total;
  }
}

}

int pa_build_sketch_csr(pa_ctx *c, const uint64_t *d_sorted_hash, const uint32_t *d_sorted_genome, uint64_t n_cand,
                        uint32_t n_genomes, uint64_t *d_hashes, uint64_t cap_hashes, uint64_t *d_off,
                        uint64_t *h_total) {
  if (n_cand == 0) {
    PA_HIP(hipMemsetAsync(d_off, 0, (uint64_t)(n_genomes + 1) * sizeof(uint64_t), c->stream));
    *h_total = 0;
    return PA_OK;
  }
  PA_TRY(c->flags.reserve(2 * n_cand * sizeof(uint32_t)));
  uint32_t *d_flags = c->flags.as<uint32_t>();
  uint32_t *d_pos = d_flags + n_cand;
  uint64_t *d_total = c->counters.as<uint64_t>() + 1;
  const uint32_t grid = ceil_div_u64(n_cand, kThreads);
  hipLaunchKernelGGL(head_flags_kernel, dim3(grid), dim3(kThreads), 0, c->stream, d_sorted_hash, d_sorted_genome,
                     n_cand, d_flags);
  PA_TRY(pa_exclusive_scan_u32(c, d_flags, d_pos, n_cand, d_total));
  PA_HIP(hipMemcpyAsync(c->h_pinned, d_total, sizeof(uint64_t), hipMemcpyDeviceToHost, c->stream));
  PA_HIP(hipStreamSynchronize(c->stream));
  *h_total = c->h_pinned[0];
  hipLaunchKernelGGL(compact_csr_kernel, dim3(grid), dim3(kThreads), 0, c->stream, d_sorted_hash, d_sorted_genome,
                     d_flags, d_pos, n_cand, n_genomes, *h_total <= cap_hashes ? cap_hashes : 0ULL, d_hashes, d_off);
  PA_HIP(hipGetLastError());
  if (*h_total > cap_hashes) {
    pa_set_error("sketch output needs %llu hashes, caller gave room for %llu", (unsigned long long)*h_total,
                 (unsigned long long)cap_hashes);
    return PA_E_CAPACITY;
  }
  return PA_OK;
}
```

pyani_plus_amd/csrc/sketch_lds.hip:

```cpp
#include <algorithm>

#include "pa_internal.h"

namespace {

constexpr int kSortThreads = 1024;
constexpr int kSortWaves = kSortThreads / 64;

__device__ __forceinline__ uint32_t wave_incl_scan(uint32_t v, uint32_t lane) {
#pragma unroll
  for (int o = 1; o < 64; o <<= 1) {
    const uint32_t t = __shfl_up(v, o, 64);
    if (lane >= (uint32_t)o) v += t;
  }
  return v;
}

constexpr uint32_t kBuckets = kSortThreads;
constexpr uint32_t kBucketCap = 48;

__global__ __launch_bounds__(kSortThreads) void genome_sort_kernel(uint64_t *__restrict__ regions,
                                                                   const uint64_t *__restrict__ region_off,
                                                                   const uint32_t *__restrict__ cursor,
                                                                   uint32_t *__restrict__ uniq, uint32_t key_shift,
                                                                   uint32_t key_mult) {
  extern __shared__ uint64_t s_key[];
  __shared__ uint32_t s_wave[kSortWaves];
  __shared__ uint32_t s_count[kBuckets], s_cursor[kBuckets];
  __shared__ uint32_t s_longest;
  const uint32_t tid = threadIdx.x, lane = tid & 63u, wave = tid >> 6;
  const uint32_t g = blockIdx.x;
  uint64_t *__restrict__ region = regions + region_off[g];
  const uint32_t room = (uint32_t)(region_off[g + 1] - region_off[g]);
  const uint32_t n = min(cursor[g], room);
  if (n == 0) {
    if (tid == 0) uniq[g] = 0;
    return;
  }
  auto bucket_of = [&](uint64_t key) -> uint32_t {
    const uint32_t b = (uint32_t)(((key >> key_shift) * (uint64_t)key_mult) >> 32);
    return b < kBuckets ? b : kBuckets - 1u;
  };
  s_count[tid] = 0;
  if (tid == 0) s_longest = 0;
  __syncthreads();
  for (uint32_t i = tid; i < n; i += kSortThreads) atomicAdd(&s_count[bucket_of(region[i])], 1u);
  __syncthreads();
  const uint32_t my_count = s_count[tid];
  {
    const uint32_t incl = wave_incl_scan(my_count, lane);
    if (lane == 63) s_wave[wave] = incl;
    uint32_t longest = my_count;
#pragma unroll
    for (int o = 32; o > 0; o >>= 1) longest = max(longest, (uint32_t)__shfl_xor(longest, o, 64));
    if (lane == 0) atomicMax(&s_longest, longest);
    __syncthreads();
    uint32_t base = 0;
    for (int w = 0; w < (int)wave; ++w) base += s_wave[w];
    s_cursor[tid] = base + incl - my_count;
  }
  __syncthreads();
  const uint32_t my_start = s_cursor[tid];
  const bool by_buckets = s_longest <= kBucketCap;
  __syncthreads();
  if (by_buckets) {
    for (uint32_t i = tid; i < n; i += kSortThreads) {
      const uint64_t key = region[i];
      s_key[atomicAdd(&s_cursor[bucket_of(key)], 1u)] = key;
    }
    __syncthreads();
    for (uint32_t i = 1; i < my_count; ++i) {
      const uint64_t key = s_key[my_start + i];
      uint32_t j = i;
      while (j > 0 && s_key[my_start + j - 1] > key) {
        s_key[my_start + j] = s_key[my_start + j - 1];
        --j;
      }
      s_key[my_start + j] = key;
    }
    __syncthreads();
  }
  uint32_t np2 = 2;
  while (np2 < n) np2 <<= 1;
  if (!by_buckets) {
    for (uint32_t i = tid; i < np2; i += kSortThreads) s_key[i] = i < n ? region[i] : ~0ULL;
    __syncthreads();
  }
  for (uint32_t k = 2; !by_buckets && k <= np2; k <<= 1) {
    for (uint32_t j = k >> 1; j > 0; j >>= 1) {
      for (uint32_t t = tid; t < (np2 >> 1); t += kSortThreads) {
        const uint32_t i = 2u * t - (t & (j - 1u));
        const uint32_t l = i + j;
        const uint64_t a = s_key[i], b = s_key[l];
        const bool up = (i & k) == 0u;
        if ((a > b) == up) {
          s_key[i] = b;
          s_key[l] = a;
        }
      }
      __syncthreads();
    }
  }
  const uint32_t per = (n + kSortThreads - 1u) / kSortThreads;
  const uint32_t beg = min(tid * per, n), end = min(beg + per, n);
  uint32_t heads = 0;
  for (uint32_t i = beg; i < end; ++i) heads += (i == 0 || s_key[i] != s_key[i - 1]) ? 1u : 0u;
  const uint32_t incl = wave_incl_scan(heads, lane);
  if (lane == 63) s_wave[wave] = incl;
  __syncthreads();
  uint32_t base = 0, total = 0;
  for (int w = 0; w < kSortWaves; ++w) {
    const uint32_t x = s_wave[w];
    if (w < (int)wave) base += x;
    total += x;
  }
  uint32_t pos = base + incl - heads;
  for (uint32_t i = beg; i < end; ++i) {
    const uint64_t v = s_key[i];
    if (i == 0 || v != s_key[i - 1]) region[pos++] = v;
  }
  if (tid == 0) uniq[g] = total;
}

__global__ __launch_bounds__(kSortThreads) void offsets_kernel(const uint32_t *__restrict__ uniq, uint32_t n,
                                                               uint64_t *__restrict__ off, uint64_t *__restrict__ total) {
  __shared__ uint32_t s_wave[kSortWaves];
  const uint32_t tid = threadIdx.x, lane = tid & 63u, wave = tid >> 6;
  uint64_t carry = 0;
  for (uint32_t i0 = 0; i0 < n; i0 += kSortThreads) {
    const uint32_t i = i0 + tid;
    const uint32_t v = i < n ? uniq[i] : 0u;
    const uint32_t incl = wave_incl_scan(v, lane);
    if (lane == 63) s_wave[wave] = incl;
    __syncthreads();
    uint32_t base = 0, sum = 0;
    for (int w = 0; w < kSortWaves; ++w) {
      const uint32_t x = s_wave[w];
      if (w < (int)wave) base += x;
      sum += x;
    }
    if (i < n) off[i] = carry + base + incl - v;
    carry += sum;
    __syncthreads();
  }
  if (tid == 0) {
    off[n] = carry;
    *total = carry;
  }
}

__global__ __launch_bounds__(256) void gather_kernel(const uint64_t *__restrict__ regions,
                                                     const uint64_t *__restrict__ region_off,
                                                     const uint64_t *__restrict__ off, uint64_t *__restrict__ hashes) {
  const uint32_t g = blockIdx.x;
  const uint64_t *__restrict__ src = regions + region_off[g];
  const uint64_t o = off[g];
  const uint32_t n = (uint32_t)(off[g + 1] - o);
  for (uint32_t i = threadIdx.x; i < n; i += 256) hashes[o + i] = src[i];
}

}

int pa_sketch_from_regions(pa_ctx *c, uint64_t *d_regions, const uint64_t *d_region_off, const uint32_t *d_cursor,
                           const uint32_t *d_overflow, uint32_t n_genomes, uint32_t longest_region, uint64_t max_hash,
                           uint64_t *d_hashes, uint64_t cap_hashes, uint64_t *d_off, uint64_t *h_total,
                           bool *h_overflow) {
  PA_REQUIRE(longest_region <= kLdsSortMax, "LDS sort: region of %u candidates exceeds %u", longest_region, kLdsSortMax);
  uint32_t np2 = 2;
  while (np2 < longest_region) np2 <<= 1;
  const uint32_t lds_bytes = np2 * (uint32_t)sizeof(uint64_t);
  PA_TRY(c->flags.reserve((uint64_t)n_genomes * sizeof(uint32_t)));
  uint32_t *d_uniq = c->flags.as<uint32_t>();
  uint64_t *d_total = c->counters.as<uint64_t>() + 1;
  PA_HIP(hipFuncSetAttribute(reinterpret_cast<const void *>(genome_sort_kernel),
                             hipFuncAttributeMaxDynamicSharedMemorySize, (int)lds_bytes));
  const int key_bits = max_hash ? 64 - __builtin_clzll(max_hash) : 1;
  const uint32_t key_shift = key_bits > 32 ? (uint32_t)key_bits - 32u : 0u;
  const uint64_t top = (max_hash >> key_shift) + 1;
  const uint32_t key_mult = (uint32_t)std::min<uint64_t>(((uint64_t)kBuckets << 32) / top, 0xffffffffull);
  hipLaunchKernelGGL(genome_sort_kernel, dim3(n_genomes), dim3(kSortThreads), lds_bytes, c->stream, d_regions,
                     d_region_off, d_cursor, d_uniq, key_shift, key_mult);
  hipLaunchKernelGGL(offsets_kernel, dim3(1), dim3(kSortThreads), 0, c->stream, d_uniq, n_genomes, d_off, d_total);
  PA_HIP(hipGetLastError());
  PA_HIP(hipMemcpyAsync(c->h_pinned, d_total, sizeof(uint64_t), hipMemcpyDeviceToHost, c->stream));
  PA_HIP(hipMemcpyAsync(c->h_pinned + 1, d_overflow, sizeof(uint32_t), hipMemcpyDeviceToHost, c->stream));
  PA_HIP(hipStreamSynchronize(c->stream));
  *h_overflow = (uint32_t)c->h_pinned[1] != 0u;
  if (*h_overflow) return PA_OK;
  *h_total = c->h_pinned[0];
  if (*h_total > cap_hashes) {
    pa_set_error("sketch output needs %llu hashes, caller gave room for %llu", (unsigned long long)*h_total,
                 (unsigned long long)cap_hashes);
    return PA_E_CAPACITY;
  }
  if (*h_total)
    hipLaunchKernelGGL(gather_kernel, dim3(n_genomes), dim3(256), 0, c->stream, d_regions, d_region_off, d_off,
                       d_hashes);
  PA_HIP(hipGetLastError());
  return PA_OK;
}
```

pyani_plus_amd/engine.py:

```python

from __future__ import annotations

import ctypes as C
from dataclasses import dataclass, field

import numpy as np

from . import _capi
from ._capi import HipBackendError, check


def max_hash_for_scaled(scaled: int) -> int:
    return int(_capi.load_library().pa_max_hash(int(scaled)))


@dataclass
class HostArena:

    packed: np.ndarray
    mask: np.ndarray
    genome_start: np.ndarray
    residues: list[int] = field(default_factory=list)
    records: list[int] = field(default_factory=list)
    invalid: list[int] = field(default_factory=list)
    contig_start: np.ndarray | None = None
    contig_len: np.ndarray | None = None
    contig_genome: np.ndarray | None = None
    pinned_packed: "object" = None
    ambig_pos: np.ndarray | None = None
    ambig_byte: np.ndarray | None = None

    @property
    def n_genomes(self) -> int:
        return len(self.genome_start) - 1

    @property
    def arena_bases(self) -> int:
        return int(self.genome_start[-1])


def _text_ambiguous(lib, text: bytes, fasta: bool, at_most: int | None = None) -> tuple[np.ndarray, np.ndarray]:
    if not len(text) or at_most == 0:
        return np.zeros(0, np.uint64), np.zeros(0, np.uint8)
    if at_most is None:
        at_most = int(lib.pa_text_ambiguous(text, len(text), int(fasta), None, None, 0))
        if at_most < 0:
            raise HipBackendError(f"pa_text_ambiguous failed: {_capi.last_error()}")
        if at_most == 0:
            return np.zeros(0, np.uint64), np.zeros(0, np.uint8)
    pos, byte = np.zeros(at_most, dtype=np.uint64), np.zeros(at_most, dtype=np.uint8)
    n = int(lib.pa_text_ambiguous(text, len(text), int(fasta), pos.ctypes.data, byte.ctypes.data, at_most))
    if n < 0 or n > at_most:
        raise HipBackendError(f"pa_text_ambiguous failed: {_capi.last_error() if n < 0 else f'{n} residues against a bound of {at_most}'}")
    return pos[:n].copy(), byte[:n].copy()


def pack_genomes(texts: list[bytes], *, fasta: bool = True) -> HostArena:
    lib = _capi.load_library()
    bounds = [int(lib.pa_pack_bound(len(t))) for t in texts]
    total = sum(bounds)
    packed = np.zeros(total // 16, dtype=np.uint32)
    mask = np.zeros(total // 32, dtype=np.uint32)
    starts = np.zeros(len(texts) + 1, dtype=np.uint64)
    residues, records, invalid = [], [], []
    c_start, c_len, c_genome = [], [], []
    a_pos, a_byte = [], []
    pos = 0
    for g, text in enumerate(texts):
        nb, nr, nrec, ninv = C.c_uint64(0), C.c_uint64(0), C.c_uint64(0), C.c_uint64(0)
        buf = bytes(text) if len(text) else None
        p_ptr = packed.ctypes.data + (pos // 16) * 4
        m_ptr = mask.ctypes.data + (pos // 32) * 4
        if fasta:
            st = lib.pa_pack_fasta(buf, len(text), p_ptr, m_ptr, bounds[g], C.byref(nb), C.byref(nr), C.byref(nrec), C.byref(ninv))
        else:
            st = lib.pa_pack_seq(buf, len(text), p_ptr, m_ptr, bounds[g], C.byref(nb), C.byref(ninv))
            nr.value, nrec.value = len(text), 1
        check(st, "pa_pack_fasta" if fasta else "pa_pack_seq")
        if fasta and nrec.value:
            rs = np.zeros(int(nrec.value), dtype=np.uint64)
            rl = np.zeros(int(nrec.value), dtype=np.uint64)
            lib.pa_fasta_records(buf, len(text), rs.ctypes.data, rl.ctypes.data, int(nrec.value))
            c_start.extend((rs + np.uint64(pos)).tolist())
            c_len.extend(rl.tolist())
            c_genome.extend([g] * int(nrec.value))
        elif not fasta:
            c_start.append(pos)
            c_len.append(len(text))
            c_genome.append(g)
        if ninv.value:
            ap, ab = _text_ambiguous(lib, buf, fasta, at_most=int(ninv.value))
            a_pos.append(ap + np.uint64(pos))
            a_byte.append(ab)
        starts[g] = pos
        pos += int(nb.value)
        residues.append(int(nr.value))
        records.append(int(nrec.value))
        invalid.append(int(ninv.value))
    starts[len(texts)] = pos
    return HostArena(
        packed[: pos // 16].copy(), mask[: pos // 32].copy(), starts, residues, records, invalid,
        np.array(c_start, dtype=np.uint64), np.array(c_len, dtype=np.uint32), np.array(c_genome, dtype=np.uint32),
        ambig_pos=np.concatenate(a_pos) if a_pos else np.zeros(0, np.uint64), ambig_byte=np.concatenate(a_byte) if a_byte else np.zeros(0, np.uint8),
    )


@dataclass
class LoadedFasta:

    path: str
    status: int
    message: str
    md5: str
    length: int
    records: int
    invalid: int
    description: str
    gzip: bool


def load_fasta_files(paths, threads: int = 0, *, pinned: bool = False) -> tuple[list[LoadedFasta], HostArena]:
    import os

    lib = _capi.load_library()
    paths = [str(p) for p in paths]
    n = len(paths)
    if threads <= 0:
        threads = int(lib.pa_host_cpu_budget())
    arr = (C.c_char_p * max(n, 1))(*[p.encode() for p in paths])
    batch = C.c_void_p()
    check(lib.pa_fasta_batch_load(arr, n, threads, C.byref(batch)), "pa_fasta_batch_load")
    try:
        infos: list[LoadedFasta] = []
        ok_residues, ok_records, ok_invalid = [], [], []
        rec_tables = []
        for i, path in enumerate(paths):
            md5 = C.create_string_buffer(33)
            nres, nrec, ninv, nb, nt = (C.c_uint64(0) for _ in range(5))
            desc, msg = C.c_char_p(), C.c_char_p()
            gz = C.c_int(0)
            st = lib.pa_fasta_batch_info(batch, i, md5, C.byref(nres), C.byref(nrec), C.byref(ninv), C.byref(nb), C.byref(nt), C.byref(desc), C.byref(msg), C.byref(gz))
            infos.append(
                LoadedFasta(path, st, (msg.value or b"").decode(errors="replace"), md5.value.decode(), int(nres.value), int(nrec.value),
                            int(ninv.value), (desc.value or b"").decode(errors="replace"), bool(gz.value))
            )
            if st == 0:
                ok_residues.append(int(nres.value))
                ok_records.append(int(nrec.value))
                ok_invalid.append(int(ninv.value))
                rs_p, rl_p, rn = C.POINTER(C.c_uint64)(), C.POINTER(C.c_uint64)(), C.c_uint64(0)
                lib.pa_fasta_batch_records(batch, i, C.byref(rs_p), C.byref(rl_p), C.byref(rn))
                k_rec = int(rn.value)
                rec_tables.append((np.ctypeslib.as_array(rs_p, (k_rec,)).copy(), np.ctypeslib.as_array(rl_p, (k_rec,)).copy()) if k_rec else (np.zeros(0, np.uint64), np.zeros(0, np.uint64)))
        total = int(lib.pa_fasta_batch_arena_bases(batch))
        pinned_packed = None
        if pinned:
            import torch

            pinned_packed = torch.empty(max(total // 16, 1), dtype=torch.int32, pin_memory=torch.cuda.is_available())
            packed = pinned_packed.numpy().view(np.uint32)
        else:
            packed = np.empty(max(total // 16, 1), dtype=np.uint32)
        mask = np.empty(max(total // 32, 1), dtype=np.uint32)
        starts_all = np.zeros(n + 1, dtype=np.uint64)
        check(lib.pa_fasta_batch_copy_arena(batch, packed.ctypes.data, mask.ctypes.data, starts_all.ctypes.data), "pa_fasta_batch_copy_arena")
        keep = [i for i, info in enumerate(infos) if info.status == 0]
        starts = np.array([starts_all[i] for i in keep] + [total], dtype=np.uint64)
        c_start = np.concatenate([rs + starts[g] for g, (rs, _rl) in enumerate(rec_tables)]) if rec_tables else np.zeros(0, np.uint64)
        c_len = np.concatenate([rl for _rs, rl in rec_tables]).astype(np.uint32) if rec_tables else np.zeros(0, np.uint32)
        c_genome = np.concatenate([np.full(len(rs), g, dtype=np.uint32) for g, (rs, _rl) in enumerate(rec_tables)]) if rec_tables else np.zeros(0, np.uint32)
        n_amb = int(lib.pa_fasta_batch_ambiguous(batch, None, None, 0))
        a_pos, a_byte = np.zeros(max(n_amb, 0), dtype=np.uint64), np.zeros(max(n_amb, 0), dtype=np.uint8)
        if n_amb > 0:
            lib.pa_fasta_batch_ambiguous(batch, a_pos.ctypes.data, a_byte.ctypes.data, n_amb)
        return infos, HostArena(
            packed[: total // 16], mask[: total // 32], starts, ok_residues, ok_records, ok_invalid,
            c_start.astype(np.uint64), c_len, c_genome, pinned_packed[: max(total // 16, 1)] if pinned_packed is not None else None,
            ambig_pos=a_pos, ambig_byte=a_byte,
        )
    finally:
        lib.pa_fasta_batch_free(batch)


@dataclass
class DeviceArena:
    packed: "object"
    mask: "object"
    genome_start: np.ndarray
    dirty: "object" = None
    ambig_pos: np.ndarray | None = None
    ambig_byte: np.ndarray | None = None

    @property
    def n_genomes(self) -> int:
        return len(self.genome_start) - 1

    @property
    def arena_bases(self) -> int:
        return int(self.genome_start[-1])


@dataclass
class PinnedArena:

    packed: "object"
    run_start: np.ndarray
    run_len: np.ndarray
    genome_start: np.ndarray

    @property
    def n_genomes(self) -> int:
        return len(self.genome_start) - 1

    @property
    def arena_bases(self) -> int:
        return int(self.genome_start[-1])


def mask_runs(mask: np.ndarray, arena_bases: int) -> tuple[np.ndarray, np.ndarray]:
    lib = _capi.load_library()
    mask = np.ascontiguousarray(mask, dtype=np.uint32)
    n = int(lib.pa_mask_runs(mask.ctypes.data, arena_bases, None, None, 0))
    if n < 0:
        raise HipBackendError("pa_mask_runs: null mask")
    start = np.empty(max(n, 1), dtype=np.uint64)
    length = np.empty(max(n, 1), dtype=np.uint64)
    got = int(lib.pa_mask_runs(mask.ctypes.data, arena_bases, start.ctypes.data, length.ctypes.data, n))
    if got != n:
        raise HipBackendError("pa_mask_runs: run count changed between calls")
    return start[:n], length[:n]


@dataclass
class DeviceSketches:

    hashes: "object"
    off: "object"
    n: int
    total: int
    host_off: np.ndarray | None = None

    def offsets_host(self) -> np.ndarray:
        if self.host_off is None:
            self.host_off = np.ascontiguousarray(self.off.cpu().numpy().astype(np.uint64))
        return self.host_off

    def sizes(self) -> np.ndarray:
        off = self.offsets_host()
        return (off[1:] - off[:-1]).astype(np.uint64)

    def to_host(self) -> list[np.ndarray]:
        off = self.offsets_host().astype(np.int64)
        flat = self.hashes[: self.total].cpu().numpy().view(np.uint64)
        return [flat[int(off[g]) : int(off[g + 1])].copy() for g in range(self.n)]


class HipEngine:

    def __init__(self, device: int = 0, *, tools: bool = False):
        self.lib = _capi.load_library(tools)
        self._check = lambda status, what: check(status, what, self.lib)
        try:
            import torch
        except ImportError as err:
            raise HipBackendError("PyTorch (ROCm build) is required for device memory") from err
        if not torch.cuda.is_available():
            raise HipBackendError("no HIP device visible to PyTorch; the HIP path has no CPU fallback")
        self.torch = torch
        self.device = torch.device("cuda", device)
        torch.cuda.set_device(self.device)
        ctx = C.c_void_p()
        self._check(self.lib.pa_ctx_create(device, C.byref(ctx)), "pa_ctx_create")
        self.ctx = ctx
        self.use_torch_stream()

    def use_torch_stream(self) -> None:
        stream = self.torch.cuda.current_stream(self.device).cuda_stream
        self._check(self.lib.pa_ctx_set_stream(self.ctx, C.c_void_p(stream)), "pa_ctx_set_stream")

    def close(self) -> None:
        if getattr(self, "ctx", None):
            self.lib.pa_ctx_destroy(self.ctx)
            self.ctx = None

    def __del__(self):
        try:
            self.close()
        except Exception:
            pass

    def device_info(self) -> dict:
        name = C.create_string_buffer(256)
        cus, mem = C.c_int(0), C.c_uint64(0)
        self._check(self.lib.pa_ctx_device_info(self.ctx, name, C.byref(cus), C.byref(mem)), "pa_ctx_device_info")
        return {"name": name.value.decode(), "compute_units": cus.value, "global_mem": mem.value}

    def sync(self) -> None:
        self._check(self.lib.pa_ctx_sync(self.ctx), "pa_ctx_sync")

    def upload(self, arena: HostArena) -> DeviceArena:
        t = self.torch
        packed = t.from_numpy(arena.packed.view(np.int32)).to(self.device)
        mask = t.from_numpy(arena.mask.view(np.int32)).to(self.device)
        return DeviceArena(packed, mask, arena.genome_start.copy(), ambig_pos=arena.ambig_pos, ambig_byte=arena.ambig_byte)

    def _set_ambiguous(self, arena: DeviceArena) -> None:
        pos = getattr(arena, "ambig_pos", None)
        n = 0 if pos is None else len(pos)
        if n:
            p = np.ascontiguousarray(pos, dtype=np.uint64)
            b = np.ascontiguousarray(arena.ambig_byte, dtype=np.uint8)
            self._check(self.lib.pa_fragani_set_ambiguous(self.ctx, arena.packed.data_ptr(), p.ctypes.data, b.ctypes.data, n), "pa_fragani_set_ambiguous")
        else:
            self._check(self.lib.pa_fragani_set_ambiguous(self.ctx, None, None, None, 0), "pa_fragani_set_ambiguous")

    def sketches_from_host(self, sketches: list[np.ndarray]) -> DeviceSketches:
        t = self.torch
        off = np.zeros(len(sketches) + 1, dtype=np.int64)
        np.cumsum([len(s) for s in sketches], out=off[1:])
        flat = np.concatenate([np.asarray(s, dtype=np.uint64) for s in sketches]) if sketches else np.empty(0, np.uint64)
        if flat.size == 0:
            flat = np.zeros(1, dtype=np.uint64)
        return DeviceSketches(
            t.from_numpy(flat.view(np.int64).copy()).to(self.device), t.from_numpy(off).to(self.device), len(sketches), int(off[-1]),
            np.ascontiguousarray(off.astype(np.uint64)),
        )

    def sketches_from_gathered(self, hashes, off, off_host: np.ndarray) -> DeviceSketches:
        hashes, off = hashes.to(self.device), off.to(self.device)
        return DeviceSketches(hashes, off, len(off_host) - 1, int(off_host[-1]), np.ascontiguousarray(off_host, dtype=np.uint64))

    def arena_dirty(self, arena: DeviceArena):
        if arena.dirty is None:
            t = self.torch
            words = (arena.arena_bases // 64 + 63) // 64
            dirty = t.empty(max(words, 1), dtype=t.int64, device=self.device)
            self._check(self.lib.pa_arena_dirty(self.ctx, arena.mask.data_ptr(), arena.arena_bases, dirty.data_ptr()), "pa_arena_dirty")
            arena.dirty = dirty
        return arena.dirty

    def sketch(self, arena: DeviceArena, k: int, scaled: int, *, max_hash: int | None = None) -> DeviceSketches:
        t = self.torch
        mh = int(max_hash) if max_hash is not None else max_hash_for_scaled(scaled)
        n = arena.n_genomes
        frac = 1.0 if mh >= 2**64 - 1 else (mh + 1) / 2.0**64
        cap = int(arena.arena_bases * frac * 1.25) + 4096
        off = t.empty(n + 1, dtype=t.int64, device=self.device)
        gs = np.ascontiguousarray(arena.genome_start, dtype=np.uint64)
        total = C.c_uint64(0)
        dirty = self.arena_dirty(arena)
        for _attempt in range(2):
            hashes = t.empty(max(cap, 1), dtype=t.int64, device=self.device)
            st = self.lib.pa_sketch(
                self.ctx, arena.packed.data_ptr(), arena.mask.data_ptr(), dirty.data_ptr(), arena.arena_bases,
                gs.ctypes.data_as(C.POINTER(C.c_uint64)), n, k, mh, hashes.data_ptr(), cap, off.data_ptr(), C.byref(total),
            )
            if st == _capi.PA_E_CAPACITY:
                cap = int(total.value)
                continue
            self._check(st, "pa_sketch")
            return DeviceSketches(hashes, off, n, int(total.value))
        raise HipBackendError("pa_sketch: capacity retry failed")

    def pin_arena(self, arena: HostArena) -> PinnedArena:
        t = self.torch
        if arena.pinned_packed is not None:
            packed = arena.pinned_packed
        else:
            packed = t.from_numpy(np.ascontiguousarray(arena.packed).view(np.int32)).pin_memory()
        start, length = mask_runs(arena.mask, int(arena.genome_start[-1]))
        return PinnedArena(packed, start, length, np.ascontiguousarray(arena.genome_start, dtype=np.uint64).copy())

    def sketch_streamed(self, host: PinnedArena, k: int, scaled: int, *, max_hash: int | None = None, arena: DeviceArena | None = None):
        t = self.torch
        mh = int(max_hash) if max_hash is not None else max_hash_for_scaled(scaled)
        n, bases = host.n_genomes, host.arena_bases
        if arena is None:
            arena = DeviceArena(
                t.empty(max(bases // 16, 1), dtype=t.int32, device=self.device),
                t.empty(max(bases // 32, 1), dtype=t.int32, device=self.device),
                host.genome_start.copy(),
            )
        if arena.dirty is None:
            arena.dirty = t.empty(max((bases // 64 + 63) // 64, 1), dtype=t.int64, device=self.device)
        frac = 1.0 if mh >= 2**64 - 1 else (mh + 1) / 2.0**64
        cap = int(bases * frac * 1.25) + 4096
        off = t.empty(n + 1, dtype=t.int64, device=self.device)
        gs = np.ascontiguousarray(host.genome_start, dtype=np.uint64)
        total = C.c_uint64(0)
        for _attempt in range(2):
            hashes = t.empty(max(cap, 1), dtype=t.int64, device=self.device)
            st = self.lib.pa_sketch_streamed(
                self.ctx, host.packed.data_ptr(), host.run_start.ctypes.data, host.run_len.ctypes.data, len(host.run_start),
                bases, gs.ctypes.data_as(C.POINTER(C.c_uint64)), n, k, mh, arena.packed.data_ptr(), arena.mask.data_ptr(),
                arena.dirty.data_ptr(), hashes.data_ptr(), cap, off.data_ptr(), C.byref(total),
            )
            if st == _capi.PA_E_CAPACITY:
                cap = int(total.value)
                continue
            self._check(st, "pa_sketch_streamed")
            return arena, DeviceSketches(hashes, off, n, int(total.value))
        raise HipBackendError("pa_sketch_streamed: capacity retry failed")

    def pair_counts(self, sk: DeviceSketches, q_range=None, s_range=None, algo: int = _capi.PA_PAIRS_AUTO):
        t = self.torch
        q0, q1 = q_range or (0, sk.n)
        s0, s1 = s_range or (0, sk.n)
        counts = t.empty((q1 - q0, s1 - s0), dtype=t.int32, device=self.device)
        h_off = sk.offsets_host()
        assert h_off.dtype == np.uint64 and len(h_off) == sk.n + 1
        self._check(
            self.lib.pa_pair_counts_ex(
                self.ctx, sk.hashes.data_ptr(), sk.off.data_ptr(), h_off.ctypes.data, sk.n, q0, q1, s0, s1, counts.data_ptr(), algo,
            ),
            "pa_pair_counts",
        )
        return counts

    def pair_dict_prepare(self, subject_hashes, n_postings: int) -> None:
        self._check(self.lib.pa_pair_dict_prepare(self.ctx, subject_hashes.data_ptr(), int(n_postings)), "pa_pair_dict_prepare")

    def ani(self, counts, sk: DeviceSketches, k: int, q_range=None, s_range=None):
        t = self.torch
        q0, q1 = q_range or (0, sk.n)
        s0, s1 = s_range or (0, sk.n)
        ident = t.empty((q1 - q0, s1 - s0), dtype=t.float64, device=self.device)
        cov = t.empty_like(ident)
        self._check(
            self.lib.pa_ani(self.ctx, counts.data_ptr(), sk.off.data_ptr(), q0, q1, s0, s1, k, ident.data_ptr(), cov.data_ptr()),
            "pa_ani",
        )
        return ident, cov

    def sketch_bottom(self, arena: DeviceArena, k: int, m: int) -> DeviceSketches:
        t = self.torch
        n = arena.n_genomes
        hashes = t.empty(max(n * m, 1), dtype=t.int64, device=self.device)
        off = t.empty(n + 1, dtype=t.int64, device=self.device)
        gs = np.ascontiguousarray(arena.genome_start, dtype=np.uint64)
        total = C.c_uint64(0)
        self._check(
            self.lib.pa_sketch_bottom(
                self.ctx, arena.packed.data_ptr(), arena.mask.data_ptr(), self.arena_dirty(arena).data_ptr(), arena.arena_bases,
                gs.ctypes.data_as(C.POINTER(C.c_uint64)), n, k, m, hashes.data_ptr(), n * m, off.data_ptr(), C.byref(total),
            ),
            "pa_sketch_bottom",
        )
        return DeviceSketches(hashes, off, n, int(total.value))

    def pair_mash(self, sk: DeviceSketches, m: int, q_range=None, s_range=None):
        t = self.torch
        q0, q1 = q_range or (0, sk.n)
        s0, s1 = s_range or (0, sk.n)
        common = t.empty((q1 - q0, s1 - s0), dtype=t.int32, device=self.device)
        denom = t.empty_like(common)
        self._check(
            self.lib.pa_pair_mash(self.ctx, sk.hashes.data_ptr(), sk.off.data_ptr(), sk.n, q0, q1, s0, s1, m, common.data_ptr(), denom.data_ptr()),
            "pa_pair_mash",
        )
        return common, denom

    def ani_mash(self, common, denom, k: int):
        t = self.torch
        out = t.empty(common.shape, dtype=t.float64, device=self.device)
        self._check(self.lib.pa_ani_mash(self.ctx, common.data_ptr(), denom.data_ptr(), common.numel(), k, out.data_ptr()), "pa_ani_mash")
        return out

    def fragani(self, arena: DeviceArena, contig_start, contig_len, contig_genome, k: int = 16, frag_len: int = 3000, ref_range=None,
                query_range=None, reuse_index: bool = False, out=None, columns_only: bool = False):
        n = arena.n_genomes
        r0, r1 = ref_range if ref_range is not None else (0, n)
        q0, q1 = query_range if query_range is not None else (0, n)
        cols = int(r1) - int(r0) if columns_only else n
        cs = np.ascontiguousarray(contig_start, dtype=np.uint64)
        cl = np.ascontiguousarray(contig_len, dtype=np.uint32)
        cg = np.ascontiguousarray(contig_genome, dtype=np.uint32)
        if out is None:
            total = np.zeros(n, dtype=np.uint32)
            matched = np.zeros((n, cols), dtype=np.uint32)
            ident_sum = np.zeros((n, cols), dtype=np.float64)
        else:
            total, matched, ident_sum = out
            assert total.shape == (n,) and matched.shape == (n, cols) == ident_sum.shape
            assert total.dtype == np.uint32 and matched.dtype == np.uint32 and ident_sum.dtype == np.float64
            assert matched.flags.c_contiguous and ident_sum.flags.c_contiguous
        flags = (_capi.PA_FRAGANI_REUSE_INDEX if reuse_index else 0) | (_capi.PA_FRAGANI_COLUMNS_ONLY if columns_only else 0)
        self._set_ambiguous(arena)
        self._check(
            self.lib.pa_fragani_ex(
                self.ctx, arena.packed.data_ptr(), arena.mask.data_ptr(), arena.arena_bases, cs.ctypes.data, cl.ctypes.data,
                cg.ctypes.data, len(cs), n, k, frag_len, int(q0), int(q1), int(r0), int(r1),
                flags, total.ctypes.data, matched.ctypes.data, ident_sum.ctypes.data,
            ),
            "pa_fragani",
        )
        return total, matched, ident_sum

    def fragani_sketch(self, arena: DeviceArena, contig_start, contig_len, contig_genome, k: int, window: int):
        cs = np.ascontiguousarray(contig_start, dtype=np.uint64)
        cl = np.ascontiguousarray(contig_len, dtype=np.uint32)
        cg = np.ascontiguousarray(contig_genome, dtype=np.uint32)
        cap = max(1024, arena.arena_bases)
        h = np.zeros(cap, dtype=np.uint32)
        wp = np.zeros(cap, dtype=np.uint32)
        ct = np.zeros(cap, dtype=np.uint32)
        n = C.c_uint64(0)
        self._set_ambiguous(arena)
        self._check(
            self.lib.pa_fragani_sketch(
                self.ctx, arena.packed.data_ptr(), arena.mask.data_ptr(), arena.arena_bases, cs.ctypes.data, cl.ctypes.data,
                cg.ctypes.data, len(cs), arena.n_genomes, k, window, h.ctypes.data, wp.ctypes.data, ct.ctypes.data, cap, C.byref(n),
            ),
            "pa_fragani_sketch",
        )
        m = int(n.value)
        return h[:m], wp[:m], ct[:m]

    def fragani_workspace(self) -> dict:
        held, peak, cap = C.c_uint64(0), C.c_uint64(0), C.c_uint64(0)
        self._check(self.lib.pa_fragani_workspace(self.ctx, C.byref(held), C.byref(peak), C.byref(cap)), "pa_fragani_workspace")
        return {"held_bytes": int(held.value), "peak_bytes": int(peak.value), "cap_bytes": int(cap.value)}

    def fragani_set_workspace_cap(self, cap_bytes: int) -> None:
        self._check(self.lib.pa_fragani_set_workspace_cap(self.ctx, int(cap_bytes)), "pa_fragani_set_workspace_cap")

    def msa_upload(self, msa: "LoadedMSA", *, chunk_bytes: int = 1 << 29) -> "DeviceMSA":
        t = self.torch
        code, bits = msa_code_table(msa.histogram)
        n, stride = msa.n_rows, msa.rows.shape[1]
        words = int(self.lib.pa_msa_plane_words(n, msa.n_cols, bits))
        planes = t.empty(max(words, 1), dtype=t.int32, device=self.device)
        nongap = t.zeros(max(n, 1), dtype=t.int32, device=self.device)
        step = max(1, int(chunk_bytes) // stride)
        for r0 in range(0, n, step):
            r1 = min(n, r0 + step)
            d_rows = t.from_numpy(msa.rows[r0:r1]).to(self.device)
            self._check(
                self.lib.pa_msa_pack(
                    self.ctx, d_rows.data_ptr(), stride, r0, r1 - r0, n, msa.n_cols, code.ctypes.data, bits, planes.data_ptr(), nongap.data_ptr()
                ),
                "pa_msa_pack",
            )
            self.sync()
        return DeviceMSA(planes, nongap, n, msa.n_cols, bits)


    def msa_pair_counts(self, dm: "DeviceMSA", q_range=None, s_range=None, *, symmetric: bool = False):
        t = self.torch
        q0, q1 = q_range or (0, dm.n_rows)
        s0, s1 = s_range or (0, dm.n_rows)
        match = t.empty((q1 - q0, s1 - s0), dtype=t.int32, device=self.device)
        both = t.empty((q1 - q0, s1 - s0), dtype=t.int32, device=self.device)
        if match.numel() == 0:
            return match, both
        self._check(
            self.lib.pa_msa_pair_counts(
                self.ctx, dm.planes.data_ptr(), dm.n_rows, dm.n_cols, dm.bits, q0, q1, s0, s1, int(bool(symmetric)), match.data_ptr(), both.data_ptr()
            ),
            "pa_msa_pair_counts",
        )
        return match, both

    def classify_edges_device(self, score, cov, *, score_edges: str = "mean", coverage_edges: str = "min", cov_min: float = 0.5):
        t = self.torch

        def on_device(m):
            if not isinstance(m, t.Tensor):
                m = t.from_numpy(np.ascontiguousarray(m, dtype=np.float64))
            return m.to(device=self.device, dtype=t.float64).contiguous()

        d_score, d_cov = on_device(score), on_device(cov)
        n = d_score.shape[0]
        if d_score.shape != (n, n) or d_cov.shape != (n, n):
            raise ValueError(f"score {tuple(d_score.shape)} and coverage {tuple(d_cov.shape)} must be square and equal")
        for name, role in ((score_edges, "score"), (coverage_edges, "coverage")):
            if name not in _capi.PA_AGG:
                raise ValueError(f"Unknown {role} aggregator {name!r}: expected one of min, max, mean")
        cap = n * (n - 1) // 2
        e_i = t.empty(cap, dtype=t.int32, device=self.device)
        e_j = t.empty(cap, dtype=t.int32, device=self.device)
        e_s = t.empty(cap, dtype=t.float64, device=self.device)
        e_c = t.empty(cap, dtype=t.float64, device=self.device)
        count = C.c_uint64(0)
        self._check(
            self.lib.pa_classify_edges(
                self.ctx, d_score.data_ptr(), d_cov.data_ptr(), n, _capi.PA_AGG[score_edges], _capi.PA_AGG[coverage_edges], float(cov_min), cap,
                e_i.data_ptr(), e_j.data_ptr(), e_s.data_ptr(), e_c.data_ptr(), C.byref(count),
            ),
            "pa_classify_edges",
        )
        m = count.value
        return e_i[:m], e_j[:m], e_s[:m], e_c[:m]

    def classify_edges(self, score, cov, *, score_edges: str = "mean", coverage_edges: str = "min", cov_min: float = 0.5):
        e_i, e_j, e_s, e_c = self.classify_edges_device(score, cov, score_edges=score_edges, coverage_edges=coverage_edges, cov_min=cov_min)
        return e_i.cpu().numpy().view(np.uint32), e_j.cpu().numpy().view(np.uint32), e_s.cpu().numpy(), e_c.cpu().numpy()

    def prof_enable(self, on: bool = True) -> None:
        self._check(self.lib.pa_prof_enable(self.ctx, int(on)), "pa_prof_enable")

    def prof_reset(self) -> None:
        self._check(self.lib.pa_prof_reset(self.ctx), "pa_prof_reset")

    def prof_get(self) -> dict[str, tuple[float, int]]:
        out = {}
        for name, idx in _capi.PROF_PHASES.items():
            ms, n = C.c_double(0), C.c_uint64(0)
            self._check(self.lib.pa_prof_get(self.ctx, idx, C.byref(ms), C.byref(n)), "pa_prof_get")
            out[name] = (ms.value, int(n.value))
        return out


def ani_host(counts: np.ndarray, q_sizes, s_sizes, k: int, *, symmetric: bool = False, threads: int = 0, out=None):
    lib = _capi.load_library()
    counts = np.ascontiguousarray(counts, dtype=np.uint32)
    nq, ns = counts.shape
    q_sizes = np.ascontiguousarray(q_sizes, dtype=np.uint64)
    s_sizes = np.ascontiguousarray(s_sizes, dtype=np.uint64)
    if out is None:
        ident = np.empty((nq, ns), dtype=np.float64)
        cov = np.empty((nq, ns), dtype=np.float64)
        null = np.empty((nq, ns), dtype=np.uint8)
    else:
        ident, cov, null = out
        assert ident.shape == cov.shape == null.shape == (nq, ns) and ident.flags.c_contiguous and cov.flags.c_contiguous
    check(
        lib.pa_ani_host(
            counts.ctypes.data, q_sizes.ctypes.data, s_sizes.ctypes.data, nq, ns, k, ident.ctypes.data, cov.ctypes.data, null.ctypes.data,
            int(bool(symmetric)), int(threads),
        ),
        "pa_ani_host",
    )
    return ident, cov, null.view(np.bool_) if null.dtype == np.uint8 else null


GAP = ord("-")


@dataclass
class LoadedMSA:

    md5: str
    titles: list[bytes]
    lengths: np.ndarray
    histogram: np.ndarray
    rows: np.ndarray
    n_cols: int

    @property
    def n_rows(self) -> int:
        return len(self.titles)


def load_msa(path, threads: int = 0) -> LoadedMSA:
    lib = _capi.load_library()
    handle = C.c_void_p()
    check(lib.pa_msa_load(str(path).encode(), int(threads), C.byref(handle)), "pa_msa_load", lib)
    try:
        n = C.c_uint32(0)
        max_len = C.c_uint64(0)
        md5 = C.create_string_buffer(33)
        hist = np.zeros(256, dtype=np.uint64)
        check(lib.pa_msa_info(handle, C.byref(n), C.byref(max_len), md5, hist.ctypes.data_as(C.POINTER(C.c_uint64))), "pa_msa_info", lib)
        titles, lengths = [], np.zeros(n.value, dtype=np.uint64)
        title, tlen, length = C.c_char_p(), C.c_uint64(0), C.c_uint64(0)
        for i in range(n.value):
            check(lib.pa_msa_record(handle, i, C.byref(title), C.byref(tlen), C.byref(length)), "pa_msa_record", lib)
            titles.append(C.string_at(title, tlen.value))
            lengths[i] = length.value
        stride = max(32, (int(max_len.value) + 31) // 32 * 32)
        rows = np.empty((n.value, stride), dtype=np.uint8)
        if n.value:
            check(lib.pa_msa_copy_rows(handle, 0, n.value, stride, rows.ctypes.data), "pa_msa_copy_rows", lib)
        return LoadedMSA(md5.value.decode(), titles, lengths, hist, rows, int(max_len.value))
    finally:
        lib.pa_msa_free(handle)


def msa_code_table(histogram) -> tuple[np.ndarray, int]:
    hist = np.asarray(histogram, dtype=np.uint64)
    present = [b for b in range(256) if hist[b] and b != GAP]
    code = np.zeros(256, dtype=np.uint8)
    for i, b in enumerate(present, start=1):
        code[b] = i
    bits = max(1, int(len(present)).bit_length())
    return code, bits


@dataclass
class DeviceMSA:
    planes: object
    nongap: object
    n_rows: int
    n_cols: int
    bits: int


def msa_metrics(match, both, n_q, n_s, threads: int = 0):
    lib = _capi.load_library()
    match = np.ascontiguousarray(match, dtype=np.uint32)
    shape = match.shape
    match = match.ravel()
    both = np.ascontiguousarray(both, dtype=np.uint32).ravel()
    n_q = np.ascontiguousarray(np.broadcast_to(np.asarray(n_q, dtype=np.uint64), shape)).ravel()
    n_s = np.ascontiguousarray(np.broadcast_to(np.asarray(n_s, dtype=np.uint64), shape)).ravel()
    n = match.size
    assert both.size == n
    ident, covq, covs = (np.empty(n, dtype=np.float64) for _ in range(3))
    aln, err = np.empty(n, dtype=np.int64), np.empty(n, dtype=np.int64)
    check(
        lib.pa_msa_metrics(
            match.ctypes.data, both.ctypes.data, n_q.ctypes.data, n_s.ctypes.data, n, ident.ctypes.data, aln.ctypes.data,
            err.ctypes.data, covq.ctypes.data, covs.ctypes.data, int(threads),
        ),
        "pa_msa_metrics",
        lib,
    )
    return ident, aln, err, covq, covs
```

Baseline: 79.21 million.

## Return host sketch offsets, drop extra sync, tighten hash screen arithmetic

Sketching now stages host metadata in reusable pinned buffers and removes one stream synchronize. It also copies the per-genome offsets back to the host during an existing sync, so later pair counting need not read them again. The murmur pre-screen is recomputed from the sum U+V with a looser limit, and 64-bit adds go through an inline v_lshl_add_u64 asm helper. The looser screen may let a few more candidates reach the exact hash check, and the inline asm ties the code to a specific ISA.

```diff
diff --git a/include/pyani_hip.h b/include/pyani_hip.h
--- a/include/pyani_hip.h
+++ b/include/pyani_hip.h
@@ -71,6 +71,9 @@
 PA_API int pa_sketch(pa_ctx *ctx, const uint32_t *d_packed, const uint32_t *d_mask, const uint64_t *d_dirty,
               uint64_t arena_bases, const uint64_t *h_genome_start, uint32_t n_genomes, uint32_t k, uint64_t max_hash,
               uint64_t *d_hashes, uint64_t cap_hashes, uint64_t *d_off, uint64_t *h_total);
+PA_API int pa_sketch_ex(pa_ctx *ctx, const uint32_t *d_packed, const uint32_t *d_mask, const uint64_t *d_dirty,
+                 uint64_t arena_bases, const uint64_t *h_genome_start, uint32_t n_genomes, uint32_t k, uint64_t max_hash,
+                 uint64_t *d_hashes, uint64_t cap_hashes, uint64_t *d_off, uint64_t *h_total, uint64_t *h_off);
 
 PA_API int64_t pa_mask_runs(const uint32_t *h_mask, uint64_t arena_bases, uint64_t *h_run_start, uint64_t *h_run_len,
                             uint64_t cap);
diff --git a/pyani_plus_amd/_capi.py b/pyani_plus_amd/_capi.py
--- a/pyani_plus_amd/_capi.py
+++ b/pyani_plus_amd/_capi.py
@@ -62,6 +62,10 @@
     "pa_sketch": (
         C.c_int,
         [_vp, _vp, _vp, _vp, C.c_uint64, _u64p, C.c_uint32, C.c_uint32, C.c_uint64, _vp, C.c_uint64, _vp, _u64p],
+    ),
+    "pa_sketch_ex": (
+        C.c_int,
+        [_vp, _vp, _vp, _vp, C.c_uint64, _u64p, C.c_uint32, C.c_uint32, C.c_uint64, _vp, C.c_uint64, _vp, _u64p, _vp],
     ),
     "pa_read_sigs": (C.c_int, [C.POINTER(C.c_char_p), C.c_uint32, C.c_uint32, C.c_uint64, C.c_uint32, C.POINTER(_vp)]),
     "pa_sig_batch_info": (C.c_int, [_vp, C.c_uint32, _u64p, C.POINTER(C.c_char_p)]),
diff --git a/pyani_plus_amd/csrc/capi.hip b/pyani_plus_amd/csrc/capi.hip
--- a/pyani_plus_amd/csrc/capi.hip
+++ b/pyani_plus_amd/csrc/capi.hip
@@ -93,6 +93,8 @@
     for (auto &pr : ph.pending) { (void)hipEventDestroy(pr.first); (void)hipEventDestroy(pr.second); }
   for (hipEvent_t e : c->event_pool) (void)hipEventDestroy(e);
   if (c->h_pinned) (void)hipHostFree(c->h_pinned);
+  c->sketch_stage.release();
+  c->sketch_off.release();
   if (c->copy_stream) { (void)hipStreamSynchronize(c->copy_stream); (void)hipStreamDestroy(c->copy_stream); c->copy_stream = nullptr; }
   if (c->own_stream && c->stream) (void)hipStreamDestroy(c->stream);
   delete c;
@@ -166,6 +168,13 @@
 int pa_sketch(pa_ctx *c, const uint32_t *d_packed, const uint32_t *d_mask, const uint64_t *d_dirty_in, uint64_t arena_bases,
               const uint64_t *h_genome_start, uint32_t n_genomes, uint32_t k, uint64_t max_hash, uint64_t *d_hashes,
               uint64_t cap_hashes, uint64_t *d_off, uint64_t *h_total) {
+  return pa_sketch_ex(c, d_packed, d_mask, d_dirty_in, arena_bases, h_genome_start, n_genomes, k, max_hash, d_hashes, cap_hashes,
+                      d_off, h_total, nullptr);
+}
+
+int pa_sketch_ex(pa_ctx *c, const uint32_t *d_packed, const uint32_t *d_mask, const uint64_t *d_dirty_in, uint64_t arena_bases,
+                 const uint64_t *h_genome_start, uint32_t n_genomes, uint32_t k, uint64_t max_hash, uint64_t *d_hashes,
+                 uint64_t cap_hashes, uint64_t *d_off, uint64_t *h_total, uint64_t *h_off) {
   PA_REQUIRE(c && d_off && h_total && h_genome_start, "pa_sketch: null argument");
   PA_REQUIRE((arena_bases % PA_ALIGN_BASES) == 0, "pa_sketch: arena_bases %llu is not a multiple of %u",
              (unsigned long long)arena_bases, PA_ALIGN_BASES);
@@ -175,7 +184,15 @@
   PA_HIP(hipSetDevice(c->device));
   *h_total = 0;
   const uint64_t n_blocks = arena_bases / PA_ALIGN_BASES;
-  std::vector<uint32_t> blk(n_genomes + 1);
+  const uint64_t n1 = (uint64_t)n_genomes + 1;
+  PA_TRY(c->sketch_stage.reserve(n1 * (sizeof(uint64_t) + sizeof(uint32_t))));
+  uint64_t *region_off = c->sketch_stage.as<uint64_t>();
+  uint32_t *blk = reinterpret_cast<uint32_t *>(region_off + n1);
+  uint64_t *h_off_pinned = nullptr;
+  if (h_off) {
+    PA_TRY(c->sketch_off.reserve(n1 * sizeof(uint64_t)));
+    h_off_pinned = c->sketch_off.as<uint64_t>();
+  }
   for (uint32_t g = 0; g <= n_genomes; ++g) {
     const uint64_t s = h_genome_start[g];
     PA_REQUIRE((s % PA_ALIGN_BASES) == 0 && (g == 0 || s >= h_genome_start[g - 1]) && s <= arena_bases,
@@ -185,14 +202,14 @@
   }
   PA_REQUIRE(n_blocks < (1ULL << 32), "pa_sketch: arena too large");
   PA_TRY(c->genome_blk.reserve((uint64_t)(n_genomes + 1) * sizeof(uint32_t)));
-  PA_HIP(hipMemcpyAsync(c->genome_blk.p, blk.data(), (uint64_t)(n_genomes + 1) * sizeof(uint32_t),
+  PA_HIP(hipMemcpyAsync(c->genome_blk.p, blk, (uint64_t)(n_genomes + 1) * sizeof(uint32_t),
                         hipMemcpyHostToDevice, c->stream));
   const double frac = (max_hash == UINT64_MAX) ? 1.0 : ((double)max_hash + 1.0) / 18446744073709551616.0;
   static const bool force_global = [] {
     const char *v = PA_TOOL_ENV("PA_SKETCH_SORT");
     return v && v[0] == 'g';
   }();
-  std::vector<uint64_t> region_off(n_genomes + 1, 0);
+  region_off[0] = 0;
   uint64_t longest_region = 0;
   for (uint32_t g = 0; g < n_genomes; ++g) {
     const uint64_t room = (uint64_t)((double)(h_genome_start[g + 1] - h_genome_start[g]) * frac * 1.25) + 128;
@@ -203,12 +220,11 @@
   if (use_regions) {
     PA_TRY(c->region_off.reserve((uint64_t)(n_genomes + 1) * sizeof(uint64_t)));
     PA_TRY(c->region_cursor.reserve((uint64_t)n_genomes * sizeof(uint32_t)));
-    PA_HIP(hipMemcpyAsync(c->region_off.p, region_off.data(), (uint64_t)(n_genomes + 1) * sizeof(uint64_t),
+    PA_HIP(hipMemcpyAsync(c->region_off.p, region_off, (uint64_t)(n_genomes + 1) * sizeof(uint64_t),
                           hipMemcpyHostToDevice, c->stream));
   }
   const uint64_t *d_dirty = nullptr;
   PA_TRY(pa_dirty_or_build(c, d_mask, n_blocks, d_dirty_in, &d_dirty));
-  PA_HIP(hipStreamSynchronize(c->stream));
 
   if (use_regions) {
     uint32_t *d_overflow = c->counters.as<uint32_t>() + 12;
@@ -226,10 +242,14 @@
       ProfScope prof(c, PA_PROF_SKETCH_SORT);
       const int st = pa_sketch_from_regions(c, c->cand_keys[0].as<uint64_t>(), c->region_off.as<uint64_t>(),
                                             c->region_cursor.as<uint32_t>(), d_overflow, n_genomes,
-                                            (uint32_t)longest_region, max_hash, d_hashes, cap_hashes, d_off, h_total, &overflow);
+                                            (uint32_t)longest_region, max_hash, d_hashes, cap_hashes, d_off, h_total, &overflow,
+                                            h_off_pinned);
       if (st != PA_OK) return st;
     }
-    if (!overflow) return PA_OK;
+    if (!overflow) {
+      if (h_off) memcpy(h_off, h_off_pinned, n1 * sizeof(uint64_t));
+      return PA_OK;
+    }
     *h_total = 0;
   }
   uint64_t cap = (uint64_t)((double)arena_bases * frac * 1.25) + 65536;
@@ -266,9 +286,11 @@
     genome_bits = (genome_bits + 7) & ~7;
     PA_TRY(pa_radix_sort_pairs(c, keys, vals, n_cand, 0, hash_bits, false, &which));
     PA_TRY(pa_radix_sort_pairs(c, keys, vals, n_cand, 0, genome_bits, true, &which));
-    int st = pa_build_sketch_csr(c, keys[which], vals[which], n_cand, n_genomes, d_hashes, cap_hashes, d_off, h_total);
+    int st = pa_build_sketch_csr(c, keys[which], vals[which], n_cand, n_genomes, d_hashes, cap_hashes, d_off, h_total,
+                                 h_off_pinned);
     if (st != PA_OK) return st;
   }
+  if (h_off) memcpy(h_off, h_off_pinned, n1 * sizeof(uint64_t));
   return PA_OK;
 }
 
diff --git a/pyani_plus_amd/csrc/kmer_hash.hip b/pyani_plus_amd/csrc/kmer_hash.hip
--- a/pyani_plus_amd/csrc/kmer_hash.hip
+++ b/pyani_plus_amd/csrc/kmer_hash.hip
@@ -46,9 +46,7 @@
   __shared__ uint32_t s_hi[LUT ? kWords : 1][256];
 
   const uint32_t tid = threadIdx.x;
-  const uint32_t max_hi = (uint32_t)(max_hash >> 32);
-  const bool take_all = max_hi == 0xffffffffu;
-  const uint32_t screen_hi = max_hi + 1u;
+  const HashScreen screen(max_hash);
   if (tid == 0) s_n = 0;
   if constexpr (LUT) {
 #pragma unroll
@@ -135,7 +133,7 @@
           (void)kMaskHi;
           uint64_t U, V;
           murmur3_pre_last_mul<K>(P, U, V);
-          if (take_all || last_mul_high_sum_plus1(U, V) <= screen_hi) {
+          if (screen.pass(U, V)) {
             const uint64_t X = U * kF2, Y = V * kF2;
             const uint64_t h = (X ^ (X >> 33)) + (Y ^ (Y >> 33));
             if (h > max_hash || ((bad[wi >> 1] >> (16 * (wi & 1) + i)) & 1u)) continue;
@@ -242,9 +240,7 @@
   __shared__ uint64_t s_lo[kWords][256];
   __shared__ uint32_t s_hi[kWords][256];
   const uint32_t tid = threadIdx.x;
-  const uint32_t max_hi = (uint32_t)(max_hash >> 32);
-  const bool take_all = max_hi == 0xffffffffu;
-  const uint32_t screen_hi = max_hi + 1u;
+  const HashScreen screen(max_hash);
   if (tid == 0) s_n = 0;
 #pragma unroll
   for (int j = 0; j < kWords; ++j) {
@@ -332,7 +328,7 @@
             }
             uint64_t U, V;
             murmur3_pre_last_mul<K>(P, U, V);
-            if (take_all || last_mul_high_sum_plus1(U, V) <= screen_hi) {
+            if (screen.pass(U, V)) {
               const uint64_t X = U * kF2, Y = V * kF2;
               const uint64_t h = (X ^ (X >> 33)) + (Y ^ (Y >> 33));
               if (h > max_hash || ((bad[wi >> 1] >> (16 * (wi & 1) + i)) & 1u)) continue;
@@ -404,10 +400,10 @@
   for (uint32_t i = 0; i < 4; ++i) {
     if (i >= nblocks) break;
     h1 ^= rotl64(P[2 * i], 31) * kC2;
-    h1 = rotl64(h1, 27) + h2;
+    h1 = add64(rotl64(h1, 27), h2);
     h1 = times5_plus(h1, 0x52dce729ULL);
     h2 ^= rotl64(P[2 * i + 1], 33) * kC1;
-    h2 = rotl64(h2, 31) + h1;
+    h2 = add64(rotl64(h2, 31), h1);
     h2 = times5_plus(h2, 0x38495ab5ULL);
   }
   uint64_t t1 = 0, t2 = 0;
@@ -490,8 +486,7 @@
   }
   uint64_t U, V;
   murmur3_pre_last_mul_rt(P, k, U, V);
-  const uint32_t max_hi = (uint32_t)(max_hash >> 32);
-  if (max_hi != 0xffffffffu && last_mul_high_sum_plus1(U, V) > max_hi + 1u) continue;
+  if (!HashScreen(max_hash).pass(U, V)) continue;
   const uint64_t X = U * kF2, Y = V * kF2;
   const uint64_t h = (X ^ (X >> 33)) + (Y ^ (Y >> 33));
   if (h > max_hash) continue;
@@ -508,6 +503,19 @@
   }
   }
 }
+
+#ifdef PA_TOOLS
+__global__ __launch_bounds__(kThreads) void hash_screen_kernel(const uint64_t *__restrict__ U, const uint64_t *__restrict__ V,
+                                                               uint64_t n, uint64_t max_hash, uint32_t *__restrict__ pass,
+                                                               uint64_t *__restrict__ hash) {
+  const uint64_t i = (uint64_t)blockIdx.x * kThreads + threadIdx.x;
+  if (i >= n) return;
+  const uint64_t u = U[i], v = V[i];
+  const uint64_t X = u * kF2, Y = v * kF2;
+  pass[i] = HashScreen(max_hash).pass(u, v) ? 1u : 0u;
+  hash[i] = (X ^ (X >> 33)) + (Y ^ (Y >> 33));
+}
+#endif
 
 }
 
@@ -569,3 +577,17 @@
   }
 #undef PA_K_CASE
 }
+
+#ifdef PA_TOOLS
+extern "C" PA_API int pa_tool_hash_screen(pa_ctx *c, const uint64_t *d_U, const uint64_t *d_V, uint64_t n, uint64_t max_hash,
+                                          uint32_t *d_pass, uint64_t *d_hash) {
+  PA_REQUIRE(c && (n == 0 || (d_U && d_V && d_pass && d_hash)), "pa_tool_hash_screen: null argument");
+  PA_REQUIRE(n < (1ULL << 31), "pa_tool_hash_screen: %llu pairs are too many for one launch", (unsigned long long)n);
+  if (n == 0) return PA_OK;
+  PA_HIP(hipSetDevice(c->device));
+  hipLaunchKernelGGL(hash_screen_kernel, dim3(ceil_div_u64(n, kThreads)), dim3(kThreads), 0, c->stream, d_U, d_V, n, max_hash,
+                     d_pass, d_hash);
+  PA_HIP(hipGetLastError());
+  return PA_OK;
+}
+#endif
diff --git a/pyani_plus_amd/csrc/murmur_dev.h b/pyani_plus_amd/csrc/murmur_dev.h
--- a/pyani_plus_amd/csrc/murmur_dev.h
+++ b/pyani_plus_amd/csrc/murmur_dev.h
@@ -44,6 +44,12 @@
 
 constexpr uint64_t kF1 = 0xff51afd7ed558ccdULL, kF2 = 0xc4ceb9fe1a85ec53ULL;
 
+__device__ __forceinline__ uint64_t add64(uint64_t a, uint64_t b) {
+  uint64_t t;
+  asm("v_lshl_add_u64 %0, %1, 0, %2" : "=v"(t) : "v"(a), "v"(b));
+  return t;
+}
+
 template <int K, int N>
 __device__ __forceinline__ void murmur3_pre_last_mul(const uint64_t (&P)[N], uint64_t &U, uint64_t &V) {
   static_assert(N >= (K + 7) / 8, "one first product per 8-byte word of the k-mer");
@@ -57,12 +63,12 @@
     if (i == 0) {
       h1 = times5_plus(rotl64(h1, 27), 5ULL * 42ULL + 0x52dce729ULL);
     } else {
-      h1 = rotl64(h1, 27) + h2;
+      h1 = add64(rotl64(h1, 27), h2);
       h1 = times5_plus(h1, 0x52dce729ULL);
     }
     const uint64_t k2 = rotl64(P[2 * i + 1], 33) * kC1;
     h2 ^= k2;
-    h2 = rotl64(h2, 31) + h1;
+    h2 = add64(rotl64(h2, 31), h1);
     h2 = times5_plus(h2, 0x38495ab5ULL);
   }
   if constexpr (tail > 8) h2 ^= rotl64(P[2 * nblocks + 1], 33) * kC1;
@@ -75,11 +81,19 @@
   V = h2;
 }
 
-__device__ __forceinline__ uint32_t last_mul_high_sum_plus1(uint64_t U, uint64_t V) {
-  constexpr uint32_t c0 = (uint32_t)kF2, c1 = (uint32_t)(kF2 >> 32);
-  const uint32_t u0 = (uint32_t)U, u1 = (uint32_t)(U >> 32), v0 = (uint32_t)V, v1 = (uint32_t)(V >> 32);
-  return (__umulhi(u0, c0) + __umulhi(v0, c0) + 1u) + ((u0 + v0) * c1 + (u1 + v1) * c0);
-}
+struct HashScreen {
+  uint32_t limit;
+  bool take_all;
+  __device__ __forceinline__ explicit HashScreen(uint64_t max_hash)
+      : limit((uint32_t)(max_hash >> 32) + 2u), take_all((uint32_t)(max_hash >> 32) >= 0xfffffffeu) {}
+  static __device__ __forceinline__ uint32_t high_word_plus1(uint64_t U, uint64_t V) {
+    constexpr uint32_t c0 = (uint32_t)kF2, c1 = (uint32_t)(kF2 >> 32);
+    const uint64_t W = U + V;
+    const uint32_t w0 = (uint32_t)W, w1 = (uint32_t)(W >> 32);
+    return __umulhi(w0, c0) + w0 * c1 + (w1 * c0 + 1u);
+  }
+  __device__ __forceinline__ bool pass(uint64_t U, uint64_t V) const { return take_all || high_word_plus1(U, V) <= limit; }
+};
 
 template <int K, int N>
 __device__ __forceinline__ uint64_t murmur3_from_products(const uint64_t (&P)[N]) {
diff --git a/pyani_plus_amd/csrc/pa_internal.h b/pyani_plus_amd/csrc/pa_internal.h
--- a/pyani_plus_amd/csrc/pa_internal.h
+++ b/pyani_plus_amd/csrc/pa_internal.h
@@ -83,6 +83,33 @@
   void release() {
     if (p) (void)hipFree(p);
     if (budget) budget->held -= bytes;
+    p = nullptr;
+    bytes = 0;
+  }
+  template <typename T>
+  T *as() const { return reinterpret_cast<T *>(p); }
+};
+
+struct PinnedBuf {
+  void *p = nullptr;
+  uint64_t bytes = 0;
+  int reserve(uint64_t want) {
+    if (want <= bytes) return PA_OK;
+    const uint64_t sz = want + want / 4 + 256;
+    if (p) (void)hipHostFree(p);
+    p = nullptr;
+    bytes = 0;
+    hipError_t e = hipHostMalloc(&p, sz, hipHostMallocDefault);
+    if (e != hipSuccess) {
+      pa_set_error("hipHostMalloc(%llu) failed: %s", (unsigned long long)sz, hipGetErrorString(e));
+      p = nullptr;
+      return PA_E_NOMEM;
+    }
+    bytes = sz;
+    return PA_OK;
+  }
+  void release() {
+    if (p) (void)hipHostFree(p);
     p = nullptr;
     bytes = 0;
   }
@@ -118,6 +145,7 @@
   DevBuf cls_i, cls_j, cls_score, cls_cov;
   void *frag_work = nullptr;
   uint64_t *h_pinned = nullptr;
+  PinnedBuf sketch_stage, sketch_off;
   bool prof_on = false;
   ProfPhase prof[PA_PROF_NPHASES];
   std::vector<hipEvent_t> event_pool;
@@ -152,11 +180,12 @@
 constexpr uint32_t kLdsSortMax = 16384;
 int pa_sketch_from_regions(pa_ctx *c, uint64_t *d_regions, const uint64_t *d_region_off, const uint32_t *d_cursor,
                            const uint32_t *d_overflow, uint32_t n_genomes, uint32_t longest_region, uint64_t max_hash,
-                           uint64_t *d_hashes, uint64_t cap_hashes, uint64_t *d_off, uint64_t *h_total, bool *h_overflow);
+                           uint64_t *d_hashes, uint64_t cap_hashes, uint64_t *d_off, uint64_t *h_total, bool *h_overflow,
+                           uint64_t *h_off_pinned = nullptr);
 
 int pa_build_sketch_csr(pa_ctx *c, const uint64_t *d_sorted_hash, const uint32_t *d_sorted_genome,
                         uint64_t n_cand, uint32_t n_genomes, uint64_t *d_hashes, uint64_t cap_hashes,
-                        uint64_t *d_off, uint64_t *h_total);
+                        uint64_t *d_off, uint64_t *h_total, uint64_t *h_off_pinned = nullptr);
 
 int pa_pairs_bitrow(pa_ctx *c, const uint64_t *d_hashes, const uint64_t *d_off, uint32_t n, uint64_t total,
                     uint32_t q0, uint32_t q1, uint32_t s0, uint32_t s1, uint32_t *d_counts);
diff --git a/pyani_plus_amd/csrc/sketch_build.hip b/pyani_plus_amd/csrc/sketch_build.hip
--- a/pyani_plus_amd/csrc/sketch_build.hip
+++ b/pyani_plus_amd/csrc/sketch_build.hip
@@ -1,3 +1,5 @@
+#include <algorithm>
+
 #include "pa_internal.h"
 
 namespace {
@@ -35,10 +37,11 @@
 
 int pa_build_sketch_csr(pa_ctx *c, const uint64_t *d_sorted_hash, const uint32_t *d_sorted_genome, uint64_t n_cand,
                         uint32_t n_genomes, uint64_t *d_hashes, uint64_t cap_hashes, uint64_t *d_off,
-                        uint64_t *h_total) {
+                        uint64_t *h_total, uint64_t *h_off_pinned) {
   if (n_cand == 0) {
     PA_HIP(hipMemsetAsync(d_off, 0, (uint64_t)(n_genomes + 1) * sizeof(uint64_t), c->stream));
     *h_total = 0;
+    if (h_off_pinned) std::fill(h_off_pinned, h_off_pinned + n_genomes + 1, (uint64_t)0);
     return PA_OK;
   }
   PA_TRY(c->flags.reserve(2 * n_cand * sizeof(uint32_t)));
@@ -60,5 +63,9 @@
                  (unsigned long long)cap_hashes);
     return PA_E_CAPACITY;
   }
+  if (h_off_pinned) {
+    PA_HIP(hipMemcpyAsync(h_off_pinned, d_off, (uint64_t)(n_genomes + 1) * sizeof(uint64_t), hipMemcpyDeviceToHost, c->stream));
+    PA_HIP(hipStreamSynchronize(c->stream));
+  }
   return PA_OK;
 }
diff --git a/pyani_plus_amd/csrc/sketch_lds.hip b/pyani_plus_amd/csrc/sketch_lds.hip
--- a/pyani_plus_amd/csrc/sketch_lds.hip
+++ b/pyani_plus_amd/csrc/sketch_lds.hip
@@ -164,7 +164,7 @@
 int pa_sketch_from_regions(pa_ctx *c, uint64_t *d_regions, const uint64_t *d_region_off, const uint32_t *d_cursor,
                            const uint32_t *d_overflow, uint32_t n_genomes, uint32_t longest_region, uint64_t max_hash,
                            uint64_t *d_hashes, uint64_t cap_hashes, uint64_t *d_off, uint64_t *h_total,
-                           bool *h_overflow) {
+                           bool *h_overflow, uint64_t *h_off_pinned) {
   PA_REQUIRE(longest_region <= kLdsSortMax, "LDS sort: region of %u candidates exceeds %u", longest_region, kLdsSortMax);
   uint32_t np2 = 2;
   while (np2 < longest_region) np2 <<= 1;
@@ -184,6 +184,8 @@
   PA_HIP(hipGetLastError());
   PA_HIP(hipMemcpyAsync(c->h_pinned, d_total, sizeof(uint64_t), hipMemcpyDeviceToHost, c->stream));
   PA_HIP(hipMemcpyAsync(c->h_pinned + 1, d_overflow, sizeof(uint32_t), hipMemcpyDeviceToHost, c->stream));
+  if (h_off_pinned)
+    PA_HIP(hipMemcpyAsync(h_off_pinned, d_off, (uint64_t)(n_genomes + 1) * sizeof(uint64_t), hipMemcpyDeviceToHost, c->stream));
   PA_HIP(hipStreamSynchronize(c->stream));
   *h_overflow = (uint32_t)c->h_pinned[1] != 0u;
   if (*h_overflow) return PA_OK;
diff --git a/pyani_plus_amd/engine.py b/pyani_plus_amd/engine.py
--- a/pyani_plus_amd/engine.py
+++ b/pyani_plus_amd/engine.py
@@ -349,17 +349,19 @@
         gs = np.ascontiguousarray(arena.genome_start, dtype=np.uint64)
         total = C.c_uint64(0)
         dirty = self.arena_dirty(arena)
+        host_off = np.empty(n + 1, dtype=np.uint64)
         for _attempt in range(2):
             hashes = t.empty(max(cap, 1), dtype=t.int64, device=self.device)
-            st = self.lib.pa_sketch(
+            st = self.lib.pa_sketch_ex(
                 self.ctx, arena.packed.data_ptr(), arena.mask.data_ptr(), dirty.data_ptr(), arena.arena_bases,
                 gs.ctypes.data_as(C.POINTER(C.c_uint64)), n, k, mh, hashes.data_ptr(), cap, off.data_ptr(), C.byref(total),
+                host_off.ctypes.data,
             )
             if st == _capi.PA_E_CAPACITY:
                 cap = int(total.value)
                 continue
-            self._check(st, "pa_sketch")
-            return DeviceSketches(hashes, off, n, int(total.value))
+            self._check(st, "pa_sketch_ex")
+            return DeviceSketches(hashes, off, n, int(total.value), host_off)
         raise HipBackendError("pa_sketch: capacity retry failed")
 
     def pin_arena(self, arena: HostArena) -> PinnedArena:
```

Result: faster. 82.12 million, median of 6 (+3.7%).
